# ilovin/lstm_ctc_ocr

Hardware: AMD Instinct MI355X
Metric: captcha images/sec training (32x256, bs=64/GPU) (higher is better)
Workload: dtype bf16; 1 GPU; VGG-7 + BiLSTM(256) + CTC train step, H=32 W=256, 10-char labels, C=64, bs=64/GPU (BASELINE.json configs[1]), Adam lr 1e-4 wd 1e-5 clip 10; global_batch=64, parallelism=dp1, hipgraph=True

## Files before the change

include/ocr_hip.h:

```cpp
#ifndef OCR_HIP_H
#define OCR_HIP_H
#include <stddef.h>
#ifdef __cplusplus
extern "C" {
#endif

enum { OCR_STATUS_OK = 0, OCR_STATUS_MEMOPS = 1, OCR_STATUS_INVALID = 2, OCR_STATUS_EXEC = 3 };

enum {
    OCR_EPI_BIAS = 1, OCR_EPI_RELU = 2, OCR_EPI_OUT_F32 = 4,
    OCR_EPI_MASK = 16, OCR_EPI_ROWSWAP = 32, OCR_EPI_ACCUM = 64
};

const char* ocr_status_string(int status);
int ocr_abi_version(void);
const char* ocr_build_id(void);

int ocr_ctc_workspace_size(int max_label_len, int max_time, int minibatch, size_t* bytes);
int ocr_ctc_loss(const float* activations, float* gradients, const int* flat_labels, const int* label_lengths,
                 const int* input_lengths, int alphabet_size, int minibatch, int max_time, int max_label_len,
                 int blank_label, float* costs, void* workspace, void* stream);
int ocr_ctc_debug(void* dbg);
int ocr_ctc_train_supported(int alphabet_size, int max_time, int max_label_len);
int ocr_ctc_loss_train(const float* activations, void* grad_ntc_bf16, float scale, const int* flat_labels,
                       const int* label_lengths, const int* input_lengths, int alphabet_size, int minibatch, int max_time,
                       int max_label_len, int blank_label, float* costs, void* stream);
int ocr_set_ctc_engine(int fast);
int ocr_ctc_long_placement(int alphabet_size, int max_time, int max_label_len);
int ocr_ctc_long_supported(int alphabet_size, int max_time, int max_label_len);
int ocr_ctc_long_workspace_size(int alphabet_size, int max_label_len, int max_time, int minibatch, size_t* bytes);
int ocr_ctc_loss_long(const float* activations, float* gradients ,
                      void* grad_ntc_bf16 , float scale,
                      const int* flat_labels, const int* label_lengths, const int* input_lengths,
                      int alphabet_size, int minibatch, int max_time, int max_label_len, int blank_label,
                      float* costs, void* workspace, size_t workspace_bytes, void* stream);
int ocr_ctc_wide_supported(int alphabet_size, int max_time, int max_label_len);
int ocr_ctc_wide_workspace_size(int alphabet_size, int max_label_len, int max_time, int minibatch, size_t* bytes);
int ocr_ctc_loss_wide(const float* activations, float* gradients ,
                      void* grad_ntc_bf16 , float scale,
                      const int* flat_labels, const int* label_lengths, const int* input_lengths,
                      int alphabet_size, int minibatch, int max_time, int max_label_len, int blank_label,
                      float* costs, void* workspace, size_t workspace_bytes, void* stream);
int ocr_ctc_score_supported(int alphabet_size, int max_time, int max_label_len, int num_candidates);
int ocr_ctc_score_workspace_size(int alphabet_size, int max_time, int minibatch, size_t* bytes);
int ocr_ctc_score(const float* activations, const int* input_lengths, const int* cand_labels, const int* cand_lengths, int sample_stride,
                  int alphabet_size, int minibatch, int max_time, int num_candidates, int max_label_len, int blank_label,
                  float* costs, int* best, float* best_cost, float* log_norm, void* workspace, size_t workspace_bytes, void* stream);
int ocr_ctc_trie_chunk_capacity(void);
int ocr_ctc_trie_supported(int alphabet_size, int max_time, int num_words);
int ocr_ctc_trie_build(const int* words, const int* lengths, int num_words, int max_label_len, int alphabet_size, int blank_label,
                       int chunk_nodes, int* num_chunks, int* num_nodes, int* nodes, int* chunk_node_start, int* chunk_word_start,
                       int* word_node, int* word_index);
int ocr_ctc_trie_workspace_size(int alphabet_size, int max_time, int minibatch, size_t* bytes);
int ocr_ctc_score_trie(const float* activations, const int* input_lengths, const int* nodes, const int* chunk_node_start,
                       const int* chunk_word_start, const int* word_node, const int* word_index, int num_chunks, int chunk_nodes,
                       int alphabet_size, int minibatch, int max_time, int num_words, int blank_label, float* costs, int* best,
                       float* best_cost, float* log_norm, void* workspace, size_t workspace_bytes, void* stream);
int ocr_ctc_topk_supported(int K, int k);
int ocr_ctc_topk_plan(int N, int K, int k, int* segments, int* segment_len);
int ocr_ctc_topk_workspace_size(int N, int K, int k, size_t* bytes);
int ocr_ctc_topk(const float* costs, long ld, int N, int K, int k, const float* log_norm, int* index, float* cost, float* log_post,
                 int* count, void* workspace, size_t workspace_bytes, void* stream);
int ocr_ctc_align_supported(int alphabet_size, int max_time, int max_label_len, int num_candidates);
int ocr_ctc_align_workspace_size(int alphabet_size, int max_time, int minibatch, int num_candidates, int max_label_len, size_t* bytes);
int ocr_ctc_align(const float* activations, const int* input_lengths, const int* cand_labels, const int* cand_lengths, int sample_stride,
                  int alphabet_size, int minibatch, int max_time, int num_candidates, int max_label_len, int blank_label,
                  int* start, int* end, float* score, float* path_cost, void* workspace, size_t workspace_bytes, void* stream);
int ocr_ctc_greedy_decode(const float* activations, const int* input_lengths, int alphabet_size, int minibatch,
                          int max_time, int blank_label, int pad_value, int* decoded, int* decoded_lengths,
                          void* stream);

int ocr_ctc_beam_workspace_size(int alphabet_size, int minibatch, int max_time, int beam_width, size_t* bytes);
int ocr_ctc_beam_decode(const float* activations, const int* input_lengths, int alphabet_size, int minibatch,
                        int max_time, int beam_width, int merge_repeated, int pad_value, int* decoded,
                        int* decoded_lengths, float* neg_log_prob, void* workspace, size_t workspace_bytes, void* stream);
int ocr_ctc_beam_kernel_choice(int alphabet_size, int beam_width);
int ocr_set_beam_engine(int engine);

int ocr_gemm_nt_bf16(const void* P, long ldp, const void* Q, long ldq, void* out, long ldo, int M, int N, int K,
                     const float* bias, const void* mask, long ldmask, int flags, int splits, int row_group,
                     int row_skip, int swap_inner, int swap_outer, void* stream);
int ocr_set_gemm_engine(int use_large_tile);
int ocr_conv3x3_bf16(const void* x, const void* wpack, void* y, int Nb, int W, int H, int Cin, int Cout,
                     const float* bias, const void* mask, int flags, void* stream);
int ocr_conv3x3_stats_rows(int Nb, int W, int H, int Cin, int Cout, int flags);
int ocr_conv3x3_bf16_stats(const void* x, const void* wpack, void* y, int Nb, int W, int H, int Cin, int Cout, const float* bias, int flags,
                           float* partials, void* stream);
int ocr_conv3x3_kernel_choice(int Nb, int W, int H, int Cin, int Cout, int flags, int kw, int kh);
int ocr_conv3x3_accum_supported(int Nb, int W, int H, int Cin, int Cout);
int ocr_conv_halo_clock_debug(void* dbg);
int ocr_conv_ws_debug(void* dbg);
int ocr_conv3x3_pool_supported(int Nb, int W, int H, int Cin, int Cout, int kw, int kh);
int ocr_conv3x3_pool_codes_supported(int Nb, int W, int H, int Cin, int Cout, int kw, int kh);
int ocr_conv3x3_relu_pool_codes_bf16(const void* x, const void* wpack, void* y, void* pooled, void* codes, int Nb, int W, int H, int Cin,
                                     int Cout, const float* bias, int kw, int kh, void* stream);
int ocr_conv3x3_relu_pool_bf16(const void* x, const void* wpack, void* y, void* pooled, int Nb, int W, int H, int Cin, int Cout,
                               const float* bias, int kw, int kh, void* stream);
int ocr_conv3x3_unpool_supported(int Nb, int W, int H, int Cin, int Cout, int kw, int kh);
int ocr_conv3x3_dgrad_unpool_bf16(const void* dy, const void* wdgrad, void* out_full, const void* codes, int Nb, int W, int H, int Cin,
                                  int Cout, int kw, int kh, int relu_mask, void* stream);
int ocr_gemm_tn_bf16(const void* A, long lda, const void* B, long ldb, float* out, long ldo, int Mk, int I, int J,
                     int row_group, int row_skip, long a_row_off, float scale, int splits, float* colsum, void* stream);
long ocr_gemm_tn_split_workspace_floats(int Mk, int I, int J);
int ocr_gemm_tn_split_bf16(const void* A, long lda, const void* B, long ldb, float* out, long ldo, int Mk, int I, int J, float scale,
                           float* colsum, float* part, long part_floats, void* stream);
int ocr_gemm_tn_batched_bf16(const void* A, long lda, long strideA, const void* B, long ldb, long strideB, float* out, long ldo,
                             long strideOut, int Mk, int I, int J, int nbatch, float scale, int splits, float* colsum,
                             long strideColsum, void* stream);
typedef struct ocr_tn_job {
    const void* A; long lda; long strideA;
    const void* B; long ldb; long strideB;
    float* out; long ldo; long strideOut;
    float* colsum; long strideColsum;
    int Mk, I, J, nbatch;
    int row_group, row_skip;
    float scale; int reserved;
} ocr_tn_job;
int ocr_gemm_tn_jobs_supported(const ocr_tn_job* jobs, int njobs);
int ocr_gemm_tn_jobs_bf16(const ocr_tn_job* jobs, int njobs, void* stream);
int ocr_set_wgrad_engine(int engine);
int ocr_conv3x3_wgrad_bf16(const void* x, const void* dy, float* dw, float* dbias, int Nb, int W, int H, int Cin,
                           int Cout, int splits, void* stream);
int ocr_conv3x3_wgrad_kernel_choice(int Nb, int W, int H, int Cin, int Cout, int has_workspace, int splits);

int ocr_conv3x3_wgrad_workspace_size(int Nb, int W, int H, int Cin, int Cout, size_t* bytes);
int ocr_conv3x3_wgrad_ws_bf16(const void* x, const void* dy, float* dw, float* dbias, int Nb, int W, int H, int Cin,
                              int Cout, int splits, void* workspace, size_t workspace_bytes, void* stream);
int ocr_conv3x3_wgrad_defer_bf16(const void* x, const void* dy, float* dw, float* dbias, int Nb, int W, int H, int Cin, int Cout,
                                 void* workspace, size_t workspace_bytes, void* job, int* job_blocks, int* deferred, void* stream);
int ocr_wgrad9_reduce_jobs(const void* jobs, int njobs, int total_blocks, void* stream);
int ocr_conv3x3_wgrad_pair_supported(const int* shape_first, const int* shape_second);
int ocr_conv3x3_wgrad_pair_defer_bf16(const void* x0, const void* dy0, float* dw0, float* dbias0, const int* shape0, void* workspace0,
                                      size_t workspace_bytes0, const void* x1, const void* dy1, float* dw1, float* dbias1, const int* shape1,
                                      void* workspace1, size_t workspace_bytes1, void* job0, void* job1, int* job_blocks0, int* job_blocks1,
                                      void* stream);

int ocr_conv1_fwd(const float* x, const float* w, const float* bias, void* y, int Nb, int W, int H, int Cout,
                  int relu, void* stream);
int ocr_conv1_wgrad(const float* x, const void* dz, float* dw, float* db, int Nb, int W, int H, int Cout,
                    void* stream);
int ocr_eltwise_bf16(int op, const void* a, const void* b, void* out, long n, void* stream);
int ocr_conv1_pool_fwd(const float* x, const float* w, const float* bias, void* p, int Nb, int W, int H, int Cout, void* stream);
int ocr_conv1_pool_fwd_train(const float* x, const float* w, const float* bias, void* p, int Nb, int W, int H, int Cout,
                             void* codes, float* zero, long zero_n, void* ones, long ones_n, void* stream);
int ocr_conv1_pool_bwd_codes(const float* x, const float* w, const float* bias, const void* dp, float* dw, float* db,
                             int Nb, int W, int H, int Cout, const void* codes, void* stream);
int ocr_conv1_pool_bwd_slab_rows(int Nb, int W, int H);
int ocr_conv1_pool_bwd_slab(const float* x, const float* w, const float* bias, const void* dp, int Nb, int W, int H, int Cout,
                            const void* codes, float* slab, void* stream);
int ocr_conv1_pool_bwd(const float* x, const float* w, const float* bias, const void* dp, float* dw, float* db, int Nb,
                       int W, int H, int Cout, void* stream);
int ocr_maxpool_fwd(const void* x, void* y, int Nb, int W, int H, int C, int kw, int kh, void* stream);
int ocr_maxpool_bwd(const void* x, const void* dy, void* dx, int Nb, int W, int H, int C, int kw, int kh,
                    int relu_mask, void* stream);
int ocr_maxpool_bwd_codes(const void* codes, const void* dy, void* dx, int Nb, int W, int H, int C, int kw, int kh,
                          int relu_mask, void* stream);
size_t ocr_bn_workspace_bytes(long M, int C);
int ocr_bn_train_fwd(const void* x, void* y, const float* gamma, const float* beta, float* save_mean,
                     float* save_rstd, long M, int C, float eps, int relu, void* workspace, const void* residual, void* stream);
int ocr_bn_train_bwd(const void* x, const void* y, const void* dy, void* dx, const float* gamma,
                     const float* save_mean, const float* save_rstd, float* dgamma, float* dbeta, long M, int C,
                     int relu, void* workspace, void* stream);
int ocr_bn_train_fwd2(const void* x, void* y, const float* gamma, const float* beta, float* save_mean, float* save_rstd, long M, int C,
                      float eps, int relu, void* workspace, const void* residual, int partial_rows, void* pooled, void* stream);
int ocr_bn_train_bwd2(const void* x, const void* y, const void* dy, void* dx, const float* gamma, const float* save_mean,
                      const float* save_rstd, float* dgamma, float* dbeta, long M, int C, int relu, void* workspace, int pooled_dy,
                      int partial_rows, void* stream);
int ocr_bn_train_fwd_codes(const void* x, const float* gamma, const float* beta, float* save_mean, float* save_rstd, long M, int C,
                           float eps, int relu, void* workspace, int partial_rows, void* pooled, void* codes, void* stream);
int ocr_bn_train_bwd_codes(const void* x, const void* codes, const void* dy, void* dx, const float* gamma, const float* save_mean,
                           const float* save_rstd, float* dgamma, float* dbeta, long M, int C, int relu, void* workspace, void* stream);
int ocr_bn_train_bwd_codes_col(const void* x, const void* codes, const void* col, int Nb, int W, int HC, void* dy_pooled_out, void* dx,
                               const float* gamma, const float* save_mean, const float* save_rstd, float* dgamma, float* dbeta, long M,
                               int C, int relu, void* workspace, void* stream);
int ocr_conv3x3_bnbwd_rows(int Nb, int W, int H, int Cin, int Cout);
int ocr_conv3x3_dgrad_bnbwd_bf16(const void* dy, const void* wdgrad, void* dx, int Nb, int W, int H, int Cin, int Cout, const void* mask_y,
                                 const void* z, const float* mean, const float* rstd, float* partials, void* stream);
int ocr_colsum_bf16(const void* a, float* out, long M, int C, long lda, void* stream);
int ocr_pack_transpose(const float* in, void* out, int R, int Cc, long ldin, int lstm_units, void* stream);
int ocr_pack_conv_dgrad(const float* w, void* out, int Cin, int Cout, void* stream);
int ocr_pack_jobs(const void* jobs, int njobs, int total_blocks, void* stream);
int ocr_cast_f32_bf16(const float* in, void* out, long n, void* stream);
int ocr_u8_to_unit_f32(const void* in, float* out, long n, void* stream);
int ocr_step_report(const float* costs, int n, const double* scalars, const void* word_addrs, int nwords, double* out, void* stream);
int ocr_bind_batch(const void* pixels, int pixels_are_u8, float* x, long n_pixels, const int* seq_len, int* seq_len_dst, int n_seq,
                   const int* labels, int* labels_dst, int n_labels, const int* labels_len, int* labels_len_dst, int n_labels_len,
                   void* stream);
int ocr_cast2d_f32_bf16(const float* in, long ldin, void* out, long ldout, int rows, int cols, void* stream);
int ocr_tnc_to_ntc_bf16(const float* in, void* out, int T, int N, int C, float scale, void* stream);
int ocr_conv5_col2im(const void* col, void* dx, int Nb, int W, int HC, void* stream);

int ocr_bn_infer_fwd(const void* x, void* y, const float* gamma, const float* beta, const float* mean, const float* var,
                     long M, int C, float eps, int relu, void* stream);
int ocr_bn_infer_bwd(const void* x, const void* y, const void* dy, void* dx, const float* gamma, const float* mean,
                     const float* var, float* dgamma, float* dbeta, long M, int C, float eps, int relu, void* stream);
int ocr_dropout_bf16(const void* in, void* out, long n, unsigned seed, const void* step_counter, float keep_prob, void* stream);
int ocr_avgpool_bf16(const void* src, void* dst, int Nb, int W, int H, int C, int kw, int kh, int backward, void* stream);
int ocr_subsample_bf16(const void* src, void* dst, int Nb, int W, int H, int C, int Wo, int Ho, int sw, int sh, int ow, int oh,
                       int backward, void* stream);
int ocr_softmax_f32(const float* in, float* out, long rows, int C, void* stream);

int ocr_lstm_fwd_step(const float* xproj, const void* whT_packed, const int* seq_len, void* hout, float* gates,
                      float* cell, int Nb, int T, int U, int step, float forget_bias, int ndir, void* stream);
int ocr_lstm_bwd_step(const void* wh, long ldw, long w_dir_stride, const int* seq_len, const void* dhout,
                      const float* gates, const float* cell, void* dz, float* dc_state, int Nb, int T, int U,
                      int step, int ndir, void* stream);
int ocr_lstm_seq_supported(int Nb, int U);
long ocr_lstm_seq_sync_words(int Nb, int U);
int ocr_lstm_seq_debug(void* dbg );
int ocr_lstm_seq_test_skew(int units, int at);
int ocr_lstm_fwd_seq(const float* xproj, const void* whT_packed, const int* seq_len, void* hout, float* gates,
                     float* cell, int Nb, int T, int U, float forget_bias, void* sync, void* stream);
int ocr_lstm_bwd_seq(const void* wh, long ldw, long w_dir_stride, const int* seq_len, const void* dhout,
                     const float* gates, const float* cell, void* dz, int Nb, int T, int U, void* sync, void* stream);
#define OCR_LSTM_PREPARED 1
int ocr_lstm_fwd_seq2(const float* xproj, const void* whT_packed, const int* seq_len, void* hout, float* gates,
                      float* cell, int Nb, int T, int U, float forget_bias, void* sync, int flags, void* stream);
int ocr_lstm_bwd_seq2(const void* wh, long ldw, long w_dir_stride, const int* seq_len, const void* dhout,
                      const float* gates, const float* cell, void* dz, int Nb, int T, int U, void* sync, int flags, void* stream);
int ocr_lstm_fwd_seq_x_supported(int Nb, int U, int D);
int ocr_lstm_fwd_seq_x(const void* x, const void* wxT_packed, const float* bias_packed, int D, const void* whT_packed,
                       const int* seq_len, void* hout, float* gates, float* cell, int Nb, int T, int U, float forget_bias,
                       void* sync, int flags, void* stream);
int ocr_set_lstm_proto(int proto);
int ocr_set_lstm_ksplit(int waves);
int ocr_lstm_hprev(const void* hout, const int* seq_len, void* hprev, int Nb, int T, int U, int ndir, void* stream);
int ocr_lstm_xh(const void* x, const void* hout, const int* seq_len, void* xh, int Nb, int T, int D, int U, int ndir, void* stream);
int ocr_lstm_pack_bias(const float* b_fw, const float* b_bw , float* out, int U, int ndir, void* stream);

int ocr_optim_scalar_count(void);
int ocr_optim_init(void* scalars , double lr, void* stream);
int ocr_optim_set_lr(void* scalars, double lr, int multiply, void* stream);
int ocr_optim_step(float* params, float* grads, float* state1, float* state2, long n, long reg_begin, long reg_end,
                   float weight_decay, float clip_norm, int solver, float beta1, float beta2, float eps,
                   void* scalars, void* stream);
int ocr_optim_step_guarded(float* params, float* grads, float* state1, float* state2, long n, long reg_begin, long reg_end,
                           float weight_decay, float clip_norm, int solver, float beta1, float beta2, float eps,
                           void* scalars, const void* guard_addrs, int nguard, void* stream);
int ocr_optim_step_guarded2(float* params, float* grads, float* state1, float* state2, long n, long reg_begin, long reg_end,
                            float weight_decay, float clip_norm, int solver, float beta1, float beta2, float eps,
                            void* scalars, const void* guard_addrs, int nguard, const float* drop_flag, void* stream);
int ocr_guard_flag(const void* guard_addrs, int nguard, float* flag_out, void* stream);

int ocr_captcha_synth(const int* params, int n_images, int words_per_image, int max_glyphs, const void* atlas, const int* stamp, int n_stamp,
                      void* out, int W, int out_h, int canvas_cap, int width_cap, void* stream);

int ocr_wgrad9_debug(void* dbg);

int ocr_probe_tr16(const int* addr , int* out , void* stream);
int ocr_probe_xcc(int* out , int nblocks, int threads, void* stream);
int ocr_occupy_cus(int nblocks, int threads, int lds_bytes, float us, void* stream);
int ocr_mfma_busy_probe(float* out, int nblocks, int threads , int iters, long long* clk, void* stream);

#ifdef __cplusplus
}
#endif
#endif
```

lstm_ctc_ocr_amd/_native.py:

```python
import ctypes
import os
import re

_HERE = os.path.dirname(os.path.abspath(__file__))
LIB_PATH = os.environ.get("OCR_NATIVE_LIB") or os.path.join(_HERE, "libocrhip.so")
HEADER_PATH = os.path.join(os.path.dirname(_HERE), "include", "ocr_hip.h")

EPI_BIAS, EPI_RELU, EPI_OUT_F32, EPI_MASK, EPI_ROWSWAP, EPI_ACCUM = 1, 2, 4, 16, 32, 64

_P, _I, _L, _F, _D = ctypes.c_void_p, ctypes.c_int, ctypes.c_long, ctypes.c_float, ctypes.c_double

_SIGS = {
    "ocr_abi_version": ([], _I),
    "ocr_build_id": ([], ctypes.c_char_p),
    "ocr_status_string": ([_I], ctypes.c_char_p),
    "ocr_ctc_workspace_size": ([_I, _I, _I, ctypes.POINTER(ctypes.c_size_t)], _I),
    "ocr_ctc_loss": ([_P, _P, _P, _P, _P, _I, _I, _I, _I, _I, _P, _P, _P], _I),
    "ocr_set_ctc_engine": ([_I], _I),
    "ocr_ctc_debug": ([_P], _I),
    "ocr_ctc_train_supported": ([_I, _I, _I], _I),
    "ocr_ctc_loss_train": ([_P, _P, _F, _P, _P, _P, _I, _I, _I, _I, _I, _P, _P], _I),
    "ocr_ctc_long_placement": ([_I, _I, _I], _I),
    "ocr_ctc_long_supported": ([_I, _I, _I], _I),
    "ocr_ctc_long_workspace_size": ([_I, _I, _I, _I, ctypes.POINTER(ctypes.c_size_t)], _I),
    "ocr_ctc_loss_long": ([_P, _P, _P, _F, _P, _P, _P, _I, _I, _I, _I, _I, _P, _P, ctypes.c_size_t, _P], _I),
    "ocr_ctc_wide_supported": ([_I, _I, _I], _I),
    "ocr_ctc_wide_workspace_size": ([_I, _I, _I, _I, ctypes.POINTER(ctypes.c_size_t)], _I),
    "ocr_ctc_loss_wide": ([_P, _P, _P, _F, _P, _P, _P, _I, _I, _I, _I, _I, _P, _P, ctypes.c_size_t, _P], _I),
    "ocr_ctc_score_supported": ([_I, _I, _I, _I], _I),
    "ocr_ctc_score_workspace_size": ([_I, _I, _I, ctypes.POINTER(ctypes.c_size_t)], _I),
    "ocr_ctc_score": ([_P, _P, _P, _P, _I, _I, _I, _I, _I, _I, _I, _P, _P, _P, _P, _P, ctypes.c_size_t, _P], _I),
    "ocr_ctc_trie_chunk_capacity": ([], _I),
    "ocr_ctc_trie_supported": ([_I, _I, _I], _I),
    "ocr_ctc_trie_build": ([_P, _P, _I, _I, _I, _I, _I, ctypes.POINTER(_I), ctypes.POINTER(_I), _P, _P, _P, _P, _P], _I),
    "ocr_ctc_trie_workspace_size": ([_I, _I, _I, ctypes.POINTER(ctypes.c_size_t)], _I),
    "ocr_ctc_score_trie": ([_P, _P, _P, _P, _P, _P, _P, _I, _I, _I, _I, _I, _I, _I, _P, _P, _P, _P, _P, ctypes.c_size_t, _P], _I),
    "ocr_ctc_topk_supported": ([_I, _I], _I),
    "ocr_ctc_topk_plan": ([_I, _I, _I, ctypes.POINTER(_I), ctypes.POINTER(_I)], _I),
    "ocr_ctc_topk_workspace_size": ([_I, _I, _I, ctypes.POINTER(ctypes.c_size_t)], _I),
    "ocr_ctc_topk": ([_P, _L, _I, _I, _I, _P, _P, _P, _P, _P, _P, ctypes.c_size_t, _P], _I),
    "ocr_ctc_align_supported": ([_I, _I, _I, _I], _I),
    "ocr_ctc_align_workspace_size": ([_I, _I, _I, _I, _I, ctypes.POINTER(ctypes.c_size_t)], _I),
    "ocr_ctc_align": ([_P, _P, _P, _P, _I, _I, _I, _I, _I, _I, _I, _P, _P, _P, _P, _P, ctypes.c_size_t, _P], _I),
    "ocr_ctc_greedy_decode":([_P, _P, _I, _I, _I, _I, _I, _P, _P, _P], _I),
    "ocr_ctc_beam_workspace_size": ([_I, _I, _I, _I, ctypes.POINTER(ctypes.c_size_t)], _I),
    "ocr_ctc_beam_decode": ([_P, _P, _I, _I, _I, _I, _I, _I, _P, _P, _P, _P, ctypes.c_size_t, _P], _I),
    "ocr_ctc_beam_kernel_choice": ([_I, _I], _I),
    "ocr_set_beam_engine": ([_I], _I),
    "ocr_gemm_nt_bf16": ([_P, _L, _P, _L, _P, _L, _I, _I, _I, _P, _P, _L, _I, _I, _I, _I, _I, _I, _P], _I),
    "ocr_set_gemm_engine": ([_I], _I),
    "ocr_gemm_tn_batched_bf16": ([_P, _L, _L, _P, _L, _L, _P, _L, _L, _I, _I, _I, _I, _F, _I, _P, _L, _P], _I),
    "ocr_gemm_tn_jobs_supported": ([_P, _I], _I),
    "ocr_gemm_tn_jobs_bf16": ([_P, _I, _P], _I),
    "ocr_lstm_xh": ([_P, _P, _P, _P, _I, _I, _I, _I, _I, _P], _I),
    "ocr_set_wgrad_engine": ([_I], _I),
    "ocr_conv3x3_bf16": ([_P, _P, _P, _I, _I, _I, _I, _I, _P, _P, _I, _P], _I),
    "ocr_conv_halo_clock_debug": ([_P], _I),
    "ocr_occupy_cus": ([_I, _I, _I, _F, _P], _I),
    "ocr_conv_ws_debug": ([_P], _I),
    "ocr_conv3x3_accum_supported": ([_I, _I, _I, _I, _I], _I),
    "ocr_conv3x3_kernel_choice": ([_I, _I, _I, _I, _I, _I, _I, _I], _I),
    "ocr_conv3x3_pool_supported": ([_I, _I, _I, _I, _I, _I, _I], _I),
    "ocr_conv3x3_relu_pool_bf16": ([_P, _P, _P, _P, _I, _I, _I, _I, _I, _P, _I, _I, _P], _I),
    "ocr_conv3x3_pool_codes_supported": ([_I, _I, _I, _I, _I, _I, _I], _I),
    "ocr_conv3x3_relu_pool_codes_bf16": ([_P, _P, _P, _P, _P, _I, _I, _I, _I, _I, _P, _I, _I, _P], _I),
    "ocr_gemm_tn_bf16": ([_P, _L, _P, _L, _P, _L, _I, _I, _I, _I, _I, _L, _F, _I, _P, _P], _I),
    "ocr_gemm_tn_split_workspace_floats": ([_I, _I, _I], _L),
    "ocr_gemm_tn_split_bf16": ([_P, _L, _P, _L, _P, _L, _I, _I, _I, _F, _P, _P, _L, _P], _I),
    "ocr_conv3x3_wgrad_bf16": ([_P, _P, _P, _P, _I, _I, _I, _I, _I, _I, _P], _I),
    "ocr_conv3x3_wgrad_kernel_choice": ([_I, _I, _I, _I, _I, _I, _I], _I),
    "ocr_conv3x3_wgrad_workspace_size": ([_I, _I, _I, _I, _I, ctypes.POINTER(ctypes.c_size_t)], _I),
    "ocr_conv3x3_wgrad_ws_bf16": ([_P, _P, _P, _P, _I, _I, _I, _I, _I, _I, _P, ctypes.c_size_t, _P], _I),
    "ocr_conv3x3_wgrad_defer_bf16": ([_P, _P, _P, _P, _I, _I, _I, _I, _I, _P, ctypes.c_size_t, _P, ctypes.POINTER(_I),
                                      ctypes.POINTER(_I), _P], _I),
    "ocr_conv3x3_wgrad_pair_supported": ([ctypes.POINTER(_I), ctypes.POINTER(_I)], _I),
    "ocr_conv3x3_wgrad_pair_defer_bf16": ([_P, _P, _P, _P, ctypes.POINTER(_I), _P, ctypes.c_size_t, _P, _P, _P, _P, ctypes.POINTER(_I), _P,
                                           ctypes.c_size_t, _P, _P, ctypes.POINTER(_I), ctypes.POINTER(_I), _P], _I),
    "ocr_wgrad9_reduce_jobs": ([_P, _I, _I, _P], _I),
    "ocr_conv1_fwd": ([_P, _P, _P, _P, _I, _I, _I, _I, _I, _P], _I),
    "ocr_conv1_wgrad": ([_P, _P, _P, _P, _I, _I, _I, _I, _P], _I),
    "ocr_eltwise_bf16": ([_I, _P, _P, _P, _L, _P], _I),
    "ocr_conv1_pool_fwd": ([_P, _P, _P, _P, _I, _I, _I, _I, _P], _I),
    "ocr_conv1_pool_fwd_train": ([_P, _P, _P, _P, _I, _I, _I, _I, _P, _P, _L, _P, _L, _P], _I),
    "ocr_conv1_pool_bwd_codes": ([_P, _P, _P, _P, _P, _P, _I, _I, _I, _I, _P, _P], _I),
    "ocr_conv1_pool_bwd_slab_rows": ([_I, _I, _I], _I),
    "ocr_conv1_pool_bwd_slab": ([_P, _P, _P, _P, _I, _I, _I, _I, _P, _P, _P], _I),
    "ocr_conv1_pool_bwd": ([_P, _P, _P, _P, _P, _P, _I, _I, _I, _I, _P], _I),
    "ocr_maxpool_fwd": ([_P, _P, _I, _I, _I, _I, _I, _I, _P], _I),
    "ocr_maxpool_bwd": ([_P, _P, _P, _I, _I, _I, _I, _I, _I, _I, _P], _I),
    "ocr_bn_workspace_bytes": ([_L, _I], ctypes.c_size_t),
    "ocr_bn_train_fwd": ([_P, _P, _P, _P, _P, _P, _L, _I, _F, _I, _P, _P, _P], _I),
    "ocr_bn_train_bwd": ([_P, _P, _P, _P, _P, _P, _P, _P, _P, _L, _I, _I, _P, _P], _I),
    "ocr_bn_train_fwd2": ([_P, _P, _P, _P, _P, _P, _L, _I, _F, _I, _P, _P, _I, _P, _P], _I),
    "ocr_bn_train_bwd2": ([_P, _P, _P, _P, _P, _P, _P, _P, _P, _L, _I, _I, _P, _I, _I, _P], _I),
    "ocr_maxpool_bwd_codes": ([_P, _P, _P, _I, _I, _I, _I, _I, _I, _I, _P], _I),
    "ocr_bn_train_fwd_codes": ([_P, _P, _P, _P, _P, _L, _I, _F, _I, _P, _I, _P, _P, _P], _I),
    "ocr_bn_train_bwd_codes": ([_P, _P, _P, _P, _P, _P, _P, _P, _P, _L, _I, _I, _P, _P], _I),
    "ocr_bn_train_bwd_codes_col": ([_P, _P, _P, _I, _I, _I, _P, _P, _P, _P, _P, _P, _P, _L, _I, _I, _P, _P], _I),
    "ocr_conv3x3_unpool_supported": ([_I, _I, _I, _I, _I, _I, _I], _I),
    "ocr_conv3x3_dgrad_unpool_bf16": ([_P, _P, _P, _P, _I, _I, _I, _I, _I, _I, _I, _I, _P], _I),
    "ocr_conv3x3_bnbwd_rows": ([_I, _I, _I, _I, _I], _I),
    "ocr_conv3x3_dgrad_bnbwd_bf16": ([_P, _P, _P, _I, _I, _I, _I, _I, _P, _P, _P, _P, _P, _P], _I),
    "ocr_conv3x3_stats_rows": ([_I, _I, _I, _I, _I, _I], _I),
    "ocr_conv3x3_bf16_stats": ([_P, _P, _P, _I, _I, _I, _I, _I, _P, _I, _P, _P], _I),
    "ocr_bn_infer_fwd": ([_P, _P, _P, _P, _P, _P, _L, _I, _F, _I, _P], _I),
    "ocr_bn_infer_bwd": ([_P, _P, _P, _P, _P, _P, _P, _P, _P, _L, _I, _F, _I, _P], _I),
    "ocr_dropout_bf16": ([_P, _P, _L, ctypes.c_uint, _P, _F, _P], _I),
    "ocr_avgpool_bf16": ([_P, _P, _I, _I, _I, _I, _I, _I, _I, _P], _I),
    "ocr_subsample_bf16": ([_P, _P, _I, _I, _I, _I, _I, _I, _I, _I, _I, _I, _I, _P], _I),
    "ocr_softmax_f32": ([_P, _P, _L, _I, _P], _I),
    "ocr_colsum_bf16": ([_P, _P, _L, _I, _L, _P], _I),
    "ocr_pack_transpose": ([_P, _P, _I, _I, _L, _I, _P], _I),
    "ocr_pack_conv_dgrad": ([_P, _P, _I, _I, _P], _I),
    "ocr_pack_jobs": ([_P, _I, _I, _P], _I),
    "ocr_cast_f32_bf16": ([_P, _P, _L, _P], _I),
    "ocr_u8_to_unit_f32": ([_P, _P, _L, _P], _I),
    "ocr_step_report": ([_P, _I, _P, _P, _I, _P, _P], _I),
    "ocr_bind_batch": ([_P, _I, _P, _L, _P, _P, _I, _P, _P, _I, _P, _P, _I, _P], _I),
    "ocr_captcha_synth": ([_P, _I, _I, _I, _P, _P, _I, _P, _I, _I, _I, _I, _P], _I),
    "ocr_cast2d_f32_bf16": ([_P, _L, _P, _L, _I, _I, _P], _I),
    "ocr_tnc_to_ntc_bf16": ([_P, _P, _I, _I, _I, _F, _P], _I),
    "ocr_conv5_col2im": ([_P, _P, _I, _I, _I, _P], _I),
    "ocr_lstm_fwd_step": ([_P, _P, _P, _P, _P, _P, _I, _I, _I, _I, _F, _I, _P], _I),
    "ocr_lstm_bwd_step": ([_P, _L, _L, _P, _P, _P, _P, _P, _P, _I, _I, _I, _I, _I, _P], _I),
    "ocr_lstm_seq_supported": ([_I, _I], _I),
    "ocr_lstm_seq_debug": ([_P], _I),
    "ocr_lstm_seq_test_skew": ([_I, _I], _I),
    "ocr_lstm_seq_sync_words": ([_I, _I], _L),
    "ocr_lstm_fwd_seq": ([_P, _P, _P, _P, _P, _P, _I, _I, _I, _F, _P, _P], _I),
    "ocr_lstm_bwd_seq": ([_P, _L, _L, _P, _P, _P, _P, _P, _I, _I, _I, _P, _P], _I),
    "ocr_lstm_fwd_seq2": ([_P, _P, _P, _P, _P, _P, _I, _I, _I, _F, _P, _I, _P], _I),
    "ocr_lstm_fwd_seq_x_supported": ([_I, _I, _I], _I),
    "ocr_lstm_fwd_seq_x": ([_P, _P, _P, _I, _P, _P, _P, _P, _P, _I, _I, _I, _F, _P, _I, _P], _I),
    "ocr_lstm_bwd_seq2": ([_P, _L, _L, _P, _P, _P, _P, _P, _I, _I, _I, _P, _I, _P], _I),
    "ocr_lstm_hprev": ([_P, _P, _P, _I, _I, _I, _I, _P], _I),
    "ocr_lstm_pack_bias": ([_P, _P, _P, _I, _I, _P], _I),
    "ocr_optim_scalar_count": ([], _I),
    "ocr_optim_init": ([_P, _D, _P], _I),
    "ocr_optim_set_lr": ([_P, _D, _I, _P], _I),
    "ocr_optim_step": ([_P, _P, _P, _P, _L, _L, _L, _F, _F, _I, _F, _F, _F, _P, _P], _I),
    "ocr_optim_step_guarded": ([_P, _P, _P, _P, _L, _L, _L, _F, _F, _I, _F, _F, _F, _P, _P, _I, _P], _I),
    "ocr_optim_step_guarded2": ([_P, _P, _P, _P, _L, _L, _L, _F, _F, _I, _F, _F, _F, _P, _P, _I, _P, _P], _I),
    "ocr_guard_flag": ([_P, _I, _P, _P], _I),
    "ocr_wgrad9_debug": ([_P], _I),
    "ocr_probe_tr16": ([_P, _P, _P], _I),
    "ocr_set_lstm_proto": ([_I], _I),
    "ocr_set_lstm_ksplit": ([_I], _I),
    "ocr_probe_xcc": ([_P, _I, _I, _P], _I),
    "ocr_mfma_busy_probe": ([_P, _I, _I, _I, _P, _P], _I),
}


class NativeError(RuntimeError):
    pass


def declared_symbols(header=HEADER_PATH):
    text = open(header).read()
    text = re.sub(r"/\*.*?\*/", "", text, flags=re.S)
    return sorted(set(re.findall(r"\b(ocr_[a-z0-9_]+)\s*\(", text)))


def source_build_id(csrc=os.path.join(_HERE, "csrc"), experiments=False):
    import glob
    import hashlib
    rel = [os.path.basename(f) for f in glob.glob(os.path.join(csrc, "*.hip"))]
    h = hashlib.sha256()
    for f in sorted(rel) + ["common.h", "conv_plan.h", "ctc_common.h", "Makefile"]:
        h.update(open(os.path.join(csrc, f), "rb").read())
    return h.hexdigest()[:16] + ("-exp" if experiments else "")


def build_id():
    return lib().ocr_build_id().decode()


_lib = None


def lib():
    global _lib
    if _lib is None:
        if not os.path.exists(LIB_PATH):
            raise NativeError(
                "libocrhip.so not found at %s — build it with `python -c 'import __graft_entry__ as g; g.build()'` "
                "(there is no CPU/eager fallback for the hot path)" % LIB_PATH)
        _lib = ctypes.CDLL(LIB_PATH)
        for name, (argtypes, restype) in _SIGS.items():
            fn = getattr(_lib, name)
            fn.argtypes = argtypes
            fn.restype = restype
        for env, setter in (("OCR_GEMM_ENGINE", "ocr_set_gemm_engine"), ("OCR_WGRAD_ENGINE", "ocr_set_wgrad_engine")):
            if os.environ.get(env):
                getattr(_lib, setter)(int(os.environ[env]))
    return _lib


def status_string(code):
    return lib().ocr_status_string(code).decode()


def call(name, *args):
    rc = getattr(lib(), name)(*args)
    if rc != 0:
        raise NativeError("%s failed: status %d (%s)" % (name, rc, status_string(rc)))


def ptr(t):
    return None if t is None else t.data_ptr()


def stream():
    import torch
    return torch.cuda.current_stream().cuda_stream
```

lstm_ctc_ocr_amd/csrc/gemm.hip:

```cpp
#include "conv_plan.h"
#include <string.h>

enum {
    EPI_BIAS = 1,
    EPI_RELU = 2,
    EPI_OUT_F32 = 4,
    EPI_ATOMIC = 8,
    EPI_MASK = 16,
    EPI_ROWSWAP = 32,
    EPI_ACCUM = 64,
};

struct GemmArgs {
    const bf16_t* P;
    const bf16_t* Q;
    long ldp, ldq;
    int M, N, K;
    int k_per_split;
    int grp, skip;
    int cW, cH, cC;
    void* out;
    long ldo;
    const float* bias;
    const bf16_t* mask;
// ... 60 lines not shown
                int kc = k0 + ((tid + i * 256) & 3) * 8;
                u32x4 v = {0, 0, 0, 0};
                if (pvalid[i] && kc < kend) v = *(const u32x4*)(prow[i] + k0);
                pst[i] = v;
            }
        } else {
            int tap = k0 / g.cC;
            int ci0 = k0 - tap * g.cC;
            int dw = tap / 3 - 1, dh = tap % 3 - 1;
            long shift = ((long)dw * g.cH + dh) * g.cC + ci0;
#pragma unroll
            for (int i = 0; i < NCP; ++i) {
                int ww = pw[i] + dw, hh = ph[i] + dh;
                bool ok = pvalid[i] && (unsigned)ww < (unsigned)g.cW && (unsigned)hh < (unsigned)g.cH;
                u32x4 v = {0, 0, 0, 0};
                if (ok) v = *(const u32x4*)(prow[i] + shift);
                pst[i] = v;
            }
        }
#pragma unroll
        for (int i = 0; i < NCQ; ++i) {
            int kc = k0 + ((tid + i * 256) & 3) * 8;
            u32x4 v = {0, 0, 0, 0};
            if (qvalid[i] && kc < kend) v = *(const u32x4*)(qrow[i] + k0);
            qst[i] = v;
        }
    };
    auto store_tiles = [&]() {
#pragma unroll
        for (int i = 0; i < NCP; ++i) {
            int c = tid + i * 256;
            *(u32x4*)(&Ps[(c >> 2) * LDS_ROW + (c & 3) * 8]) = pst[i];
        }
#pragma unroll
        for (int i = 0; i < NCQ; ++i) {
            int c = tid + i * 256;
            *(u32x4*)(&Qs[(c >> 2) * LDS_ROW + (c & 3) * 8]) = qst[i];
        }
    };

    f32x4 acc[FN][FM];
#pragma unroll
    for (int a = 0; a < FN; ++a)
#pragma unroll
        for (int b = 0; b < FM; ++b) acc[a][b] = (f32x4){0.f, 0.f, 0.f, 0.f};

    const int frow = lane & 15, fk = (lane >> 4) * 8;
    if (kbeg < kend) {
        load_tiles(kbeg);
        for (int k0 = kbeg; k0 < kend; k0 += 32) {
            __syncthreads();
            store_tiles();
            __syncthreads();
            if (k0 + 32 < kend) load_tiles(k0 + 32);
            bf16x8 af[FN], bfr[FM];
#pragma unroll
            for (int a = 0; a < FN; ++a)
                af[a] = *(const bf16x8*)(&Qs[(wn * 16 * FN + a * 16 + frow) * LDS_ROW + fk]);
#pragma unroll
            for (int b = 0; b < FM; ++b)
                bfr[b] = *(const bf16x8*)(&Ps[(wm * 16 * FM + b * 16 + frow) * LDS_ROW + fk]);
#pragma unroll
            for (int a = 0; a < FN; ++a)
#pragma unroll
                for (int b = 0; b < FM; ++b)
                    acc[a][b] = __builtin_amdgcn_mfma_f32_16x16x32_bf16(af[a], bfr[b], acc[a][b], 0, 0, 0);
        }
    }

    const int flags = g.flags;
    const bool add_bias = (flags & EPI_BIAS) && (!(flags & EPI_ATOMIC) || blockIdx.z == 0);
#pragma unroll
    for (int a = 0; a < FN; ++a) {
        int n = n0 + wn * 16 * FN + a * 16 + (lane >> 4) * 4;
        if (n >= g.N) continue;
        f32x4 bv = {0.f, 0.f, 0.f, 0.f};
        if (add_bias) bv = *(const f32x4*)(g.bias + n);
#pragma unroll
        for (int b = 0; b < FM; ++b) {
            int m = m0 + wm * 16 * FM + b * 16 + (lane & 15);
            if (m >= g.M) continue;
            f32x4 v = acc[a][b] + bv;
            if (flags & EPI_RELU) {
                v.x = fmaxf(v.x, 0.f); v.y = fmaxf(v.y, 0.f); v.z = fmaxf(v.z, 0.f); v.w = fmaxf(v.w, 0.f);
            }
            if (flags & EPI_MASK) {
                u32x2 mk = *(const u32x2*)(g.mask + (long)m * g.ldmask + n);
                if (!(bf_lo(mk.x) > 0.f)) v.x = 0.f;
                if (!(bf_hi(mk.x) > 0.f)) v.y = 0.f;
                if (!(bf_lo(mk.y) > 0.f)) v.z = 0.f;
                if (!(bf_hi(mk.y) > 0.f)) v.w = 0.f;
            }
            long orow = m;
            if (flags & EPI_ROWSWAP) orow = (long)(m % g.swap_inner) * g.swap_outer + m / g.swap_inner;
            if (flags & EPI_OUT_F32) {
                float* o = (float*)g.out + orow * g.ldo + n;
                if (flags & EPI_ATOMIC) {
                    atomicAdd(o + 0, v.x); atomicAdd(o + 1, v.y); atomicAdd(o + 2, v.z); atomicAdd(o + 3, v.w);
                } else if (flags & EPI_ACCUM) {
                    f32x4 old = *(f32x4*)o;
                    *(f32x4*)o = old + v;
                } else {
                    *(f32x4*)o = v;
                }
            } else {
                u32x2 pk;
                pk.x = pack_bf2(v.x, v.y);
                pk.y = pack_bf2(v.z, v.w);
                *(u32x2*)((bf16_t*)g.out + orow * g.ldo + n) = pk;
            }
        }
    }
}

template <int MODE, int FM, int FN>
static int launch_gemm(const GemmArgs& g, hipStream_t stream) {
    constexpr int BM = 32 * FM, BN = 32 * FN;
    int splits = ceil_div(g.K, g.k_per_split);
    dim3 grid(ceil_div(g.M, BM), ceil_div(g.N, BN), splits);
    gemm_nt_kernel<MODE, FM, FN><<<grid, 256, 0, stream>>>(g);
    OCR_CHECK_LAUNCH();
    return OCR_OK;
}

static int dispatch_gemm(GemmArgs& g, int mode, int splits, hipStream_t stream) {
    if (g.M <= 0 || g.N <= 0 || g.K <= 0 || (g.K & 7) || (g.N & 3)) return OCR_ERR_INVALID;
    if (!g.P || !g.Q || !g.out) return OCR_ERR_INVALID;
    if (splits < 1) splits = 1;
    int kps = ceil_div(ceil_div(g.K, splits), 32) * 32;
    g.k_per_split = kps;
    if (splits > 1) {
        if (!(g.flags & EPI_OUT_F32) || (g.flags & (EPI_RELU | EPI_MASK | EPI_ACCUM))) return OCR_ERR_INVALID;
        g.flags |= EPI_ATOMIC;
    }
    long big_blocks = (long)ceil_div(g.M, 128) * ceil_div(g.N, 128) * ceil_div(g.K, kps);
    bool big = big_blocks >= 192 && g.N >= 128;
    if (mode == 1) {
        if (g.cC % 32 || g.K != 9 * g.cC) return OCR_ERR_INVALID;
        return big ? launch_gemm<1, 4, 4>(g, stream) : launch_gemm<1, 2, 2>(g, stream);
    }
    return big ? launch_gemm<0, 4, 4>(g, stream) : launch_gemm<0, 2, 2>(g, stream);
}

int ig_try_dispatch(const void* P, long ldp, const void* Q, long ldq, void* out, long ldo, int M, int N, int K,
                    const float* bias, const void* mask, long ldmask, int flags, int mode, int grp, int skip, int cW,
                    int cH, int cC, int swap_inner, int swap_outer, hipStream_t stream);
static int g_use_igemm = 1, g_use_halo = 1;
extern int g_ig_stages;
extern "C" int ocr_set_gemm_engine(int mode) {
    if (mode < 0 || mode > 3) return OCR_ERR_INVALID;
    g_use_igemm = mode != 0; g_use_halo = mode == 1; g_ig_stages = (mode == 2) ? 2 : 3;
    return OCR_OK;
}

extern "C" int ocr_gemm_nt_bf16(const void* P, long ldp, const void* Q, long ldq, void* out, long ldo,
                                int M, int N, int K, const float* bias, const void* mask, long ldmask,
                                int flags, int splits, int row_group, int row_skip, int swap_inner,
                                int swap_outer, void* stream) {
    GemmArgs g = {};
    g.P = (const bf16_t*)P; g.Q = (const bf16_t*)Q; g.ldp = ldp; g.ldq = ldq;
    g.M = M; g.N = N; g.K = K; g.grp = row_group; g.skip = row_skip;
    g.out = out; g.ldo = ldo; g.bias = bias; g.mask = (const bf16_t*)mask; g.ldmask = ldmask;
    g.flags = flags & ~EPI_ATOMIC; g.swap_inner = swap_inner; g.swap_outer = swap_outer;
    if ((flags & EPI_BIAS) && !bias) return OCR_ERR_INVALID;
    if ((flags & EPI_MASK) && !mask) return OCR_ERR_INVALID;
    if ((flags & EPI_ROWSWAP) && (swap_inner <= 0 || swap_outer <= 0)) return OCR_ERR_INVALID;
    if (g_use_igemm && splits <= 1 && P && Q && out && M > 0 && N > 0 && K > 0) {
        int rc = ig_try_dispatch(P, ldp, Q, ldq, out, ldo, M, N, K, bias, mask, ldmask, g.flags, 0, row_group, row_skip, 0, 0, 0,
                                 swap_inner, swap_outer, (hipStream_t)stream);
        if (rc >= 0) return rc;
    }
    return dispatch_gemm(g, 0, splits, (hipStream_t)stream);
}


struct ConvKnobs {
    int ws, k2, k3, k2_cfg;
    int k2_minsteps, k2_mintiles, k2_allow_a, k2_abl, k2_nst;
    int k3_minsteps, k3_genw, k3_prio;
    int halo_nw, halo_stagger, halo_stagger_bit, halo_prio;
};
static int env_int(const char* e, int dflt) { return e ? atoi(e) : dflt; }
static ConvKnobs read_conv_knobs() {
    ConvKnobs k;
    k.ws = env_int(getenv("OCR_CONV_WS"), 1);
    k.k2 = env_int(getenv("OCR_CONV_K2"), 1);
    k.k3 = env_int(getenv("OCR_CONV_K3"), 1);
    const char* cfg = getenv("OCR_K2_CFG");
    k.k2_cfg = (cfg && (cfg[0] == 'A' || cfg[0] == 'D')) ? cfg[0] : 0;
    k.k2_minsteps = env_int(ocr_tune_env("OCR_K2_MINSTEPS"), 18);
    k.k2_mintiles = env_int(ocr_tune_env("OCR_K2_MINTILES"), 128);
    const char* tiles = ocr_tune_env("OCR_K2_TILES");
    k.k2_allow_a = !(tiles && tiles[0] == 'D');
    k.k2_abl = env_int(ocr_tune_env("OCR_K2_ABL"), 0);
    k.k2_nst = env_int(ocr_tune_env("OCR_K2_NST"), 0);
    k.k3_minsteps = env_int(ocr_tune_env("OCR_K3_MINSTEPS"), 18);
    k.k3_genw = env_int(ocr_tune_env("OCR_K3_GENW"), 1);
    k.k3_prio = env_int(ocr_tune_env("OCR_K3_PRIO"), 2);
    k.halo_nw = env_int(ocr_tune_env("OCR_HALO_NW"), 0);
    const char* st = ocr_tune_env("OCR_HALO_STAGGER");
    const char* comma = st ? strchr(st, ',') : nullptr;
    k.halo_stagger = st && atoi(st) > 0 ? atoi(st) : 0;
    k.halo_stagger_bit = comma ? atoi(comma + 1) : 32;
    k.halo_prio = env_int(ocr_tune_env("OCR_HALO_PRIO"), 1);
    return k;
}
static const ConvKnobs& conv_knobs() {
    static const ConvKnobs k = read_conv_knobs();
    return k;
}

int ocr_cu_count() {
    static int cus = 0;
    if (!cus) {
        int dev = 0; hipDeviceProp_t prop;
        if (hipGetDevice(&dev) == hipSuccess && hipGetDeviceProperties(&prop, dev) == hipSuccess && prop.multiProcessorCount > 0) cus = prop.multiProcessorCount;
    }
    return cus > 0 ? cus : 256;
}

static bool plan_ws(ConvPlan& p, const ConvKnobs& k) {
    if (!k.ws || (p.flags & ~(EPI_BIAS | EPI_RELU | EPI_MASK))) return false;
    if (p.epi_kind && (!(p.flags & EPI_RELU) || (p.flags & EPI_MASK))) return false;
    if ((p.Cout & 63) || (long)p.M * p.Cin * 2 > 0x7fffffffL || (long)p.M * p.Cout * 2 > 0x7fffffffL) return false;
    int nc, bm;
    if (p.H == 16 && p.Cin == 64) { nc = 16; bm = 256; }
    else if (p.H == 16 && p.Cin == 128) { nc = 8; bm = 128; }
    else if (p.H == 8 && p.Cin == 128) { nc = 16; bm = 128; }
    else return false;
    if (p.W % nc || p.M % bm || (p.epi_kind == CONV_EPI_POOL22 && (p.W & 1))) return false;
    const int ncu = ocr_cu_count();
    const int mtiles = p.M / bm, ntiles = p.Cout / 64;
    if (k.ws == 1 && (p.Cin != 64 || (long)mtiles * ntiles < 2L * ncu)) return false;
    int slots = ncu / ntiles;
    if (slots < 1) slots = 1;
    if (slots > mtiles) slots = mtiles;
    p.per_slot = (mtiles + slots - 1) / slots;
    p.slots = (mtiles + p.per_slot - 1) / p.per_slot;
    p.grid = p.slots * ntiles;
    p.xcd_map = (p.grid % 8 == 0 && (p.grid / 8) % ntiles == 0) ? 1 : 0;
    p.family = CONV_WS; p.ws_nc = nc; p.ws_ksplit = p.Cin == 64 ? 1 : 2;
    return true;
}

static char k2_tile(const ConvPlan& p, const ConvKnobs& k, int minsteps) {
    const long M = p.M;
    if ((p.Cin & 63) || (p.Cout & 63) || M < 4096 || p.H > 16 || p.H < 1) return 0;
    if (M * p.Cin * 2 >= 0x7fffffffL || (long)p.Cout * 9 * p.Cin * 2 >= 0x7fffffffL) return 0;
    for (int pass = 0; pass < 2; ++pass)
        for (const char c : {'A', 'D'}) {
            if (k.k2_cfg && c != k.k2_cfg) continue;
            if (!k.k2_cfg && c == 'A' && !k.k2_allow_a) continue;
            const int bn = c == 'A' ? 128 : 64;
            if (p.Cout % bn) continue;
            if (k.k2_cfg) return c;
            if (9 * (p.Cin / 64) < minsteps) return 0;
            if ((M + 255) / 256 * (p.Cout / bn) >= (pass == 0 ? 224 : k.k2_mintiles)) return c;
        }
    return 0;
}

static bool plan_k3(ConvPlan& p, const ConvKnobs& k, char tile) {
    const int H = p.H, epi = p.epi_kind;
    if (H != 2 && H != 4 && H != 8 && H != 16) return false;
    if (p.M % 256 || (p.Cin & 63) || (p.Cout & 63) || (tile == 'A' && p.Cout % 128)) return false;
    const int NC = 256 / H, PS = (NC + 2 + 7) / 8 * 8;
    const bool genw = p.W % NC != 0;
    if (genw && (H == 16 || NC + 2 + (NC + p.W - 1) / p.W > PS)) return false;
    if (genw && !k.k3_genw) return false;
    if (H == 2 && (!genw || epi == CONV_EPI_POOL12 || epi == CONV_EPI_POOL22)) return false;
    if (epi >= CONV_EPI_STATS && (p.flags & EPI_ACCUM)) return false;
    if (epi == CONV_EPI_BNBWD && (!(p.flags & EPI_MASK) || p.Cin == 64 || (H != 4 && H != 8))) return false;
    p.family = CONV_K3; p.tile = tile; p.genw = genw; p.single = H == 16 && p.Cin == 64; p.prio = k.k3_prio;
    return true;
}

static bool plan_k3_k2(ConvPlan& p, const ConvKnobs& k) {
    if (k.k3) {
        const char t = k2_tile(p, k, k.k3_minsteps >= 0 ? k.k3_minsteps : k.k2_minsteps);
        if (t && plan_k3(p, k, t)) return true;
    }
    if (p.epi_kind >= CONV_EPI_STATS) return false;
    const char t = k2_tile(p, k, k.k2_minsteps);
    if (!t) return false;
    int nst = t == 'A' ? 5 : 4;
    if ((t == 'A' && k.k2_nst == 4) || (t == 'D' && (k.k2_nst == 5 || k.k2_nst == 6))) nst = k.k2_nst;
    const int FM = t == 'A' ? 8 : 4, BN = t == 'A' ? 128 : 64;
    const int NRpad = (256 + 2 * p.H + 4 + 7) / 8 * 8;
    const int lds = 2 * NRpad * 128 + nst * BN * 128;
    if (lds > 163840 || lds < 8 * FM * 2048) return false;
#ifdef OCR_EXPERIMENTS
    if (lds + 10240 > 163840 && (k.k2_abl & 8)) return false;
#endif
    p.family = CONV_K2; p.tile = t; p.nst = nst; p.abl = k.k2_abl;
    return true;
}

static bool plan_halo(ConvPlan& p, const ConvKnobs& k) {
    const int H = p.H, Cout = p.Cout, nw = k.halo_nw;
    p.prio = k.halo_prio; p.stagger = k.halo_stagger; p.stagger_bit = k.halo_stagger_bit;
    if (nw != 8) {
        const int NR = 128 + 2 * H + 2, NRp = (NR + 32) / 32 * 32;
        const long mt4 = (p.M + 127) / 128;
        if (NRp / 32 == 5 || NRp / 32 == 6) {
            p.family = CONV_HALO; p.nw = 4; p.bn = (Cout >= 128 && mt4 * ((Cout + 127) / 128) >= 448) ? 128 : 64;
            return true;
// ... 149 lines not shown
```

lstm_ctc_ocr_amd/csrc/gemm_tn3.hip:

```cpp
#include "common.h"
#include <stdlib.h>
#include <type_traits>

struct Tn3Job {
    const bf16_t* A; long lda; long sA;
    const bf16_t* B; long ldb; long sB;
    float* out; long ldo; long sO;
    float* colsum; long sC;
    int Mk, I, J, nbatch;
    int grp, skip;
    float scale; int reserved;
};
static_assert(sizeof(Tn3Job) == 120, "mirrored by lstm_ctc_ocr_amd/ops.py (ctypes.Structure)");

__device__ u32x4 tn3_zero_page[4];

typedef const __attribute__((address_space(1))) void* gptr_t;
typedef __attribute__((address_space(3))) void* lptr_t;
typedef __attribute__((ext_vector_type(4))) short s16x4;
typedef __attribute__((ext_vector_type(8))) short s16x8;

__device__ __forceinline__ int tn3_frag_off(int cb, int lane) {
    const int g = lane >> 4, L = lane & 15;
    const int r0 = 4 * g + (L >> 2);
    const int q = cb * 2 + ((L & 3) >> 1);
    const int p = q ^ ((r0 & 7) << 1);
    return r0 * 256 + p * 16 + (L & 1) * 8;
}

template <int KH, int NST >
__device__ __forceinline__ void tn3_body(const Tn3Job& g, const int bid, unsigned char* smem) {
    constexpr int TILE = 64 * 256, STAGE = 2 * TILE, DEPTH = NST - 2;
    const int tid = threadIdx.x, lane = tid & 63;
    const int wave = __builtin_amdgcn_readfirstlane(tid >> 6);
    const int wi = (wave & 3) >> 1, wj = wave & 1;

    const int IT = g.I >> 7, JT = g.J >> 7, T = IT * JT * g.nbatch;
    int L = bid;
    if ((T & 7) == 0) L = (bid & 7) * (T >> 3) + (bid >> 3);
    int jt, it;
    if ((long)g.I >= (long)g.J) { jt = L % JT; it = (L / JT) % IT; }
    else { it = L % IT; jt = (L / IT) % JT; }
    const int bi = L / (JT * IT);
    const bf16_t* A = g.A + (long)bi * g.sA;
    const bf16_t* B = g.B + (long)bi * g.sB;
    float* out = g.out + (long)bi * g.sO;
    const int i0 = it * 128, j0 = jt * 128, Mk = g.Mk;
    const bool do_cs = g.colsum != nullptr && it == 0;
    const bf16_t* zero = (const bf16_t*)tn3_zero_page;

    const int rsub = lane >> 4, pos = lane & 15;
    const bf16_t* pa[2]; const bf16_t* pb[2];
    int mrow[2], mq[2], mr[2];
    const int grp = g.grp, dq = grp > 0 ? 64 / grp : 0, dr = grp > 0 ? 64 % grp : 0;
#pragma unroll
    for (int j = 0; j < 2; ++j) {
        const int r = (wave * 2 + j) * 4 + rsub;
        const int q = pos ^ ((r & 7) << 1);
        mrow[j] = r;
        mq[j] = grp > 0 ? r / grp : 0; mr[j] = grp > 0 ? r % grp : 0;
        pa[j] = A + i0 + q * 8;
        pb[j] = B + j0 + q * 8;
    }
    auto stage_load = [&](int buf) {
        unsigned char* sa = smem + buf * STAGE;
        unsigned char* sb = sa + TILE;
#pragma unroll
        for (int j = 0; j < 2; ++j) {
            const int m = mrow[j];
            const bf16_t* srca = zero;
            const bf16_t* srcb = zero;
            if (m < Mk) {
                srca = pa[j] + ((long)m + (long)mq[j] * g.skip) * g.lda;
                srcb = pb[j] + (long)m * g.ldb;
            }
            __builtin_amdgcn_global_load_lds((gptr_t)srca, (lptr_t)(sa + (wave * 2 + j) * 1024), 16, 0, 0);
            __builtin_amdgcn_global_load_lds((gptr_t)srcb, (lptr_t)(sb + (wave * 2 + j) * 1024), 16, 0, 0);
            mrow[j] = m + 64;
            if (grp > 0) {
                int r2 = mr[j] + dr, q2 = mq[j] + dq;
                if (r2 >= grp) { r2 -= grp; ++q2; }
                mr[j] = r2; mq[j] = q2;
            }
        }
    };

    f32x4 acc[4][4];
#pragma unroll
    for (int a = 0; a < 4; ++a)
#pragma unroll
        for (int b = 0; b < 4; ++b) acc[a][b] = (f32x4){0.f, 0.f, 0.f, 0.f};
    float cs[8] = {0.f, 0.f, 0.f, 0.f, 0.f, 0.f, 0.f, 0.f};

    const unsigned lds0 = (unsigned)(size_t)(lptr_t)smem;
    unsigned offf[8];
#pragma unroll
    for (int a = 0; a < 4; ++a) {
        offf[a] = lds0 + tn3_frag_off(wi * 4 + a, lane) + KH * 32 * 256;
        offf[4 + a] = lds0 + TILE + tn3_frag_off(wj * 4 + a, lane) + KH * 32 * 256;
    }

    const int nst = (Mk + 63) >> 6;
#pragma unroll
    for (int d = 0; d < DEPTH; ++d) stage_load(d);
    asm volatile("s_waitcnt vmcnt(0)" ::: "memory");
    __builtin_amdgcn_s_barrier();
    asm volatile("" ::: "memory");

    s16x4 flo[8], fhi[8];
    auto load = [&](int buf) {
#pragma unroll
        for (int f = 0; f < 8; ++f) {
            const unsigned ad = offf[f] + buf * STAGE;
            asm volatile("ds_read_b64_tr_b16 %0, %1" : "=v"(flo[f]) : "v"(ad));
            asm volatile("ds_read_b64_tr_b16 %0, %1 offset:4096" : "=v"(fhi[f]) : "v"(ad));
        }
    };
    auto comp = [&]() {
        asm volatile("s_waitcnt lgkmcnt(0)" ::: "memory");
        __builtin_amdgcn_sched_barrier(0);
        __builtin_amdgcn_s_setprio(KH == 1 ? 2 : 1);
        bf16x8 fr[8];
#pragma unroll
        for (int f = 0; f < 8; ++f) {
            s16x8 v = {flo[f][0], flo[f][1], flo[f][2], flo[f][3], fhi[f][0], fhi[f][1], fhi[f][2], fhi[f][3]};
            fr[f] = __builtin_bit_cast(bf16x8, v);
        }
#pragma unroll
        for (int a = 0; a < 4; ++a)
#pragma unroll
            for (int b = 0; b < 4; ++b)
                acc[a][b] = __builtin_amdgcn_mfma_f32_16x16x32_bf16(fr[a], fr[4 + b], acc[a][b], 0, 0, 0);
        __builtin_amdgcn_s_setprio(0);
        __builtin_amdgcn_sched_barrier(0);
    };
    int buf = 0;
    for (int s = 0; s < nst; ++s) {
        int nb = buf + DEPTH; if (nb >= NST) nb -= NST;
        if (KH == 0) {
            load(buf);
            stage_load(nb);
            comp();
            if (do_cs) {
                const unsigned tb = lds0 + buf * STAGE + TILE;
                const int q = tid & 15;
                u32x4 v[4];
#pragma unroll
                for (int i = 0; i < 4; ++i) {
                    const int r = (tid >> 4) + 16 * i;
                    asm volatile("ds_read_b128 %0, %1" : "=v"(v[i]) : "v"(tb + r * 256 + ((q ^ ((r & 7) << 1)) << 4)));
                }
                asm volatile("s_waitcnt lgkmcnt(0)" ::: "memory");
                __builtin_amdgcn_sched_barrier(0);
#pragma unroll
                for (int i = 0; i < 4; ++i) {
                    cs[0] += bf_lo(v[i].x); cs[1] += bf_hi(v[i].x); cs[2] += bf_lo(v[i].y); cs[3] += bf_hi(v[i].y);
                    cs[4] += bf_lo(v[i].z); cs[5] += bf_hi(v[i].z); cs[6] += bf_lo(v[i].w); cs[7] += bf_hi(v[i].w);
                }
            }
        } else {
            if (s > 0) comp();
            load(buf);
            stage_load(nb);
        }
        asm volatile("s_waitcnt vmcnt(%0)" ::"n"(4 * (DEPTH - 1)) : "memory");
        __builtin_amdgcn_sched_barrier(0);
        __builtin_amdgcn_s_barrier();
        asm volatile("" ::: "memory");
        __builtin_amdgcn_sched_barrier(0);
        buf = (buf + 1 == NST) ? 0 : buf + 1;
    }
    if (KH == 1) comp();
    asm volatile("s_waitcnt vmcnt(0)" ::: "memory");
    __syncthreads();

    {
        f32x4* mine = (f32x4*)smem + (size_t)wave * (8 * 64);
        const f32x4* theirs = (const f32x4*)smem + (size_t)(wave ^ 4) * (8 * 64);
#pragma unroll
        for (int a2 = 0; a2 < 2; ++a2)
#pragma unroll
            for (int b = 0; b < 4; ++b) mine[(a2 * 4 + b) * 64 + lane] = acc[(1 - KH) * 2 + a2][b];
        __syncthreads();
#pragma unroll
        for (int a2 = 0; a2 < 2; ++a2)
#pragma unroll
            for (int b = 0; b < 4; ++b) acc[KH * 2 + a2][b] += theirs[(a2 * 4 + b) * 64 + lane];
    }
    if (do_cs) {
        __syncthreads();
        float* red = (float*)smem;
        if (KH == 0) {
#pragma unroll
            for (int e = 0; e < 8; ++e) red[tid * 8 + e] = cs[e];
        }
        __syncthreads();
        if (tid < 128) {
            float t = 0.f;
            for (int u = tid >> 3; u < 256; u += 16) t += red[u * 8 + (tid & 7)];
            g.colsum[(long)bi * g.sC + j0 + tid] += t * g.scale;
        }
    }
    const float scale = g.scale;
    float old[2][4][4];
#pragma unroll
    for (int a2 = 0; a2 < 2; ++a2)
#pragma unroll
        for (int b = 0; b < 4; ++b)
#pragma unroll
            for (int r = 0; r < 4; ++r)
                old[a2][b][r] = __builtin_nontemporal_load(out + (long)(i0 + wi * 64 + (KH * 2 + a2) * 16 + (lane >> 4) * 4 + r) * g.ldo + j0 + wj * 64 + b * 16 + (lane & 15));
#pragma unroll
    for (int a2 = 0; a2 < 2; ++a2)
#pragma unroll
        for (int b = 0; b < 4; ++b)
#pragma unroll
            for (int r = 0; r < 4; ++r)
                out[(long)(i0 + wi * 64 + (KH * 2 + a2) * 16 + (lane >> 4) * 4 + r) * g.ldo + j0 + wj * 64 + b * 16 + (lane & 15)] =
                    old[a2][b][r] + acc[KH * 2 + a2][b][r] * scale;
}

template <int NST>
__global__ __launch_bounds__(512) __attribute__((amdgpu_waves_per_eu(2, 2))) void gemm_tn3_kernel(Tn3Job j0, Tn3Job j1, int nblk0) {
    extern __shared__ __attribute__((aligned(16))) unsigned char smem[];
    const int kh = __builtin_amdgcn_readfirstlane((int)(threadIdx.x >> 8));
    const int bid = (int)blockIdx.x;
    if (bid < nblk0) {
        if (kh == 0) tn3_body<0, NST>(j0, bid, smem); else tn3_body<1, NST>(j0, bid, smem);
    } else {
        if (kh == 0) tn3_body<0, NST>(j1, bid - nblk0, smem); else tn3_body<1, NST>(j1, bid - nblk0, smem);
    }
}

static bool tn3_covers(const Tn3Job& j) {
    if (!j.A || !j.B || !j.out || j.Mk < 256 || j.I <= 0 || j.J <= 0 || (j.I & 127) || (j.J & 127) || j.nbatch < 1) return false;
    if ((j.lda & 7) || (j.ldb & 7) || (j.sA & 7) || (j.sB & 7) || ((size_t)j.A & 15) || ((size_t)j.B & 15)) return false;
    if (j.grp < 0 || j.skip < 0 || (j.grp == 0 && j.skip != 0)) return false;
    return (long)(j.I >> 7) * (j.J >> 7) * j.nbatch <= 0x7fffffL;
}
extern "C" int ocr_gemm_tn_jobs_supported(const void* jobs, int njobs) {
    if (!jobs || njobs < 1 || njobs > 2) return 0;
    const Tn3Job* j = (const Tn3Job*)jobs;
    for (int k = 0; k < njobs; ++k) if (!tn3_covers(j[k])) return 0;
    return 1;
}
extern "C" int ocr_gemm_tn_jobs_bf16(const void* jobs, int njobs, void* stream) {
    if (!ocr_gemm_tn_jobs_supported(jobs, njobs)) return OCR_ERR_INVALID;
    const Tn3Job* j = (const Tn3Job*)jobs;
    const int t0 = (j[0].I >> 7) * (j[0].J >> 7) * j[0].nbatch;
    const int t1 = njobs > 1 ? (j[1].I >> 7) * (j[1].J >> 7) * j[1].nbatch : 0;
    static int nst = -1;
    if (nst < 0) { const char* e = getenv("OCR_TN3_NST"); nst = (e && atoi(e) == 5) ? 5 : 4; }
    const int lds = nst * 2 * 64 * 256;
    if (nst == 4) {
        if (ocr_allow_lds<gemm_tn3_kernel<4>>(lds) != hipSuccess) return OCR_ERR_EXEC;
        gemm_tn3_kernel<4><<<t0 + t1, 512, lds, (hipStream_t)stream>>>(j[0], njobs > 1 ? j[1] : j[0], t0);
    } else {
        if (ocr_allow_lds<gemm_tn3_kernel<5>>(lds) != hipSuccess) return OCR_ERR_EXEC;
        gemm_tn3_kernel<5><<<t0 + t1, 512, lds, (hipStream_t)stream>>>(j[0], njobs > 1 ? j[1] : j[0], t0);
    }
    OCR_CHECK_LAUNCH();
    return OCR_OK;
}
```

lstm_ctc_ocr_amd/csrc/igemm.hip:

```cpp
#include "common.h"
#include <stdlib.h>

enum { IG_BIAS = 1, IG_RELU = 2, IG_OUT_F32 = 4, IG_MASK = 16, IG_ROWSWAP = 32 };

struct IgArgs {
    const bf16_t* P; const bf16_t* Q;
    long ldp, ldq;
    int M, N, K;
    int grp, skip;
    int cW, cH, cC;
    void* out; long ldo;
    const float* bias; const bf16_t* mask; long ldmask;
    int flags, swap_inner, swap_outer;
};

__device__ u32x4 ig_zero_page[4];

typedef const __attribute__((address_space(1))) void* gptr_t;
typedef __attribute__((address_space(3))) void* lptr_t;

template <int BN, int MODE , int STAGES , int NW >
__global__ __launch_bounds__(64 * NW) __attribute__((amdgpu_waves_per_eu(2, 2))) void igemm_kernel(IgArgs g) {
    constexpr int BM = 32 * NW, BK = 64;
    constexpr int WAVES_N = BN / 64, WAVES_M = NW / WAVES_N;
    constexpr int WM = BM / WAVES_M;
    constexpr int FM = WM / 16, FN = 4;
    constexpr int PB = BM * BK * 2, QB = BN * BK * 2, STAGE = PB + QB;
    constexpr int QI = BN / (8 * NW);
    extern __shared__ __attribute__((aligned(16))) unsigned char smem[];

    const int tid = threadIdx.x, lane = tid & 63;
    const int wave = __builtin_amdgcn_readfirstlane(tid >> 6);
    const int wm = wave / WAVES_N, wn = wave % WAVES_N;

    const int mtiles = (g.M + BM - 1) / BM, ntiles = (g.N + BN - 1) / BN;
    const int nblk = mtiles * ntiles;
    int L = blockIdx.x;
    if ((nblk & 7) == 0) L = (L & 7) * (nblk >> 3) + (L >> 3);
    const int m0 = (L / ntiles) * BM, n0 = (L % ntiles) * BN;

    const int rsub = lane >> 3;
    const int csrc = ((lane & 7) ^ rsub) * 8;
    const bf16_t* zero = (const bf16_t*)ig_zero_page;
    const bf16_t* prow[4];
    int pw[4], ph[4];
    bool pok[4];
#pragma unroll
    for (int j = 0; j < 4; ++j) {
        int m = m0 + (wave * 4 + j) * 8 + rsub;
        pok[j] = m < g.M;
        int mm = pok[j] ? m : 0;
        if (MODE == 0) {
            long phys = (long)mm + (g.grp > 0 ? (long)(mm / g.grp) * g.skip : 0);
            prow[j] = g.P + phys * g.ldp + csrc;
            pw[j] = ph[j] = 0;
        } else {
            ph[j] = mm % g.cH;
            pw[j] = (mm / g.cH) % g.cW;
            prow[j] = g.P + (long)mm * g.cC + csrc;
        }
    }
    const bf16_t* qrow[QI];
#pragma unroll
    for (int j = 0; j < QI; ++j) {
        int n = n0 + (wave * QI + j) * 8 + rsub;
        qrow[j] = (n < g.N) ? g.Q + (long)n * g.ldq + csrc : nullptr;
    }

    auto stage_load = [&](int k0, int buf) {
        unsigned char* sp = smem + buf * STAGE;
        long shift = k0;
        int dw = 0, dh = 0;
        if (MODE == 1) {
            int tap = k0 / g.cC;
            dw = tap / 3 - 1; dh = tap % 3 - 1;
            shift = ((long)dw * g.cH + dh) * g.cC + (k0 - tap * g.cC);
        }
#pragma unroll
        for (int j = 0; j < 4; ++j) {
            bool ok = pok[j];
            if (MODE == 1) ok = ok && (unsigned)(pw[j] + dw) < (unsigned)g.cW && (unsigned)(ph[j] + dh) < (unsigned)g.cH;
            const bf16_t* src = ok ? prow[j] + shift : zero;
            __builtin_amdgcn_global_load_lds((gptr_t)src, (lptr_t)(sp + (wave * 4 + j) * 1024), 16, 0, 0);
        }
#pragma unroll
        for (int j = 0; j < QI; ++j) {
            const bf16_t* src = qrow[j] ? qrow[j] + k0 : zero;
            __builtin_amdgcn_global_load_lds((gptr_t)src, (lptr_t)(sp + PB + (wave * QI + j) * 1024), 16, 0, 0);
        }
    };

    f32x4 acc[FN][FM];
#pragma unroll
    for (int a = 0; a < FN; ++a)
#pragma unroll
        for (int b = 0; b < FM; ++b) acc[a][b] = (f32x4){0.f, 0.f, 0.f, 0.f};

    const int frow = lane & 15, fq = lane >> 4, fx = lane & 7;
    const int ntk = g.K / BK;
    constexpr int NI = 4 + QI;
    const unsigned lds0 = (unsigned)(size_t)(lptr_t)smem;
    const unsigned qoff = PB + (wn * 64 + frow) * 128 + ((fq ^ fx) << 4);
    const unsigned poff = (wm * WM + frow) * 128 + ((fq ^ fx) << 4);
    auto compute = [&](int buf) {
        const unsigned base = lds0 + buf * STAGE;
        u32x4 af[2][FN], bfr[2][FM];
#pragma unroll
        for (int kk = 0; kk < 2; ++kk) {
#pragma unroll
            for (int a = 0; a < FN; ++a)
                asm volatile("ds_read_b128 %0, %1 offset:%2" : "=v"(af[kk][a]) : "v"(base + (qoff ^ (kk * 64))), "n"(a * 2048));
#pragma unroll
            for (int b = 0; b < FM; ++b)
                asm volatile("ds_read_b128 %0, %1 offset:%2" : "=v"(bfr[kk][b]) : "v"(base + (poff ^ (kk * 64))), "n"(b * 2048));
        }
#pragma unroll
        for (int kk = 0; kk < 2; ++kk) {
            if (kk == 0) asm volatile("s_waitcnt lgkmcnt(%0)" ::"n"(FN + FM) : "memory");
            else asm volatile("s_waitcnt lgkmcnt(0)" ::: "memory");
            __builtin_amdgcn_sched_barrier(0);
#pragma unroll
            for (int a = 0; a < FN; ++a)
#pragma unroll
                for (int b = 0; b < FM; ++b)
                    acc[a][b] = __builtin_amdgcn_mfma_f32_16x16x32_bf16(__builtin_bit_cast(bf16x8, af[kk][a]),
                                                                        __builtin_bit_cast(bf16x8, bfr[kk][b]), acc[a][b], 0, 0, 0);
            __builtin_amdgcn_sched_barrier(0);
        }
    };
    if (STAGES == 2) {
        stage_load(0, 0);
        asm volatile("s_waitcnt vmcnt(0)" ::: "memory");
        __syncthreads();
        for (int t = 0; t < ntk; ++t) {
            const int cur = t & 1;
            if (t + 1 < ntk) stage_load((t + 1) * BK, cur ^ 1);
            compute(cur);
            asm volatile("s_waitcnt vmcnt(0)" ::: "memory");
            __syncthreads();
        }
    } else {
        stage_load(0, 0);
        if (ntk > 1) stage_load(BK, 1);
        int cur = 0;
        for (int t = 0; t < ntk; ++t) {
            if (t + 1 < ntk) asm volatile("s_waitcnt vmcnt(%0)" ::"n"(NI) : "memory");
            else asm volatile("s_waitcnt vmcnt(0)" ::: "memory");
            __builtin_amdgcn_s_barrier();
            asm volatile("" ::: "memory");
            if (t + 2 < ntk) { int nb = cur + 2; if (nb >= 3) nb -= 3; stage_load((t + 2) * BK, nb); }
            compute(cur);
            asm volatile("s_waitcnt lgkmcnt(0)" ::: "memory");
            cur = (cur == 2) ? 0 : cur + 1;
        }
    }

    const int flags = g.flags;
    f32x4 bv[FN];
#pragma unroll
    for (int a = 0; a < FN; ++a) {
        const int n = n0 + wn * 64 + a * 16 + (lane >> 4) * 4;
        bv[a] = (f32x4){0.f, 0.f, 0.f, 0.f};
        if ((flags & IG_BIAS) && n < g.N) bv[a] = *(const f32x4*)(g.bias + n);
    }
#pragma unroll
    for (int b = 0; b < FM; ++b) {
        const int m = m0 + wm * WM + b * 16 + (lane & 15);
        if (m >= g.M) continue;
        long orow = m;
        if (flags & IG_ROWSWAP) orow = (long)(m % g.swap_inner) * g.swap_outer + m / g.swap_inner;
#pragma unroll
        for (int a = 0; a < FN; ++a) {
            const int n = n0 + wn * 64 + a * 16 + (lane >> 4) * 4;
            if (n >= g.N) continue;
            f32x4 v = acc[a][b] + bv[a];
            if (flags & IG_RELU) {
                v.x = fmaxf(v.x, 0.f); v.y = fmaxf(v.y, 0.f); v.z = fmaxf(v.z, 0.f); v.w = fmaxf(v.w, 0.f);
            }
            if (flags & IG_MASK) {
                u32x2 mk = *(const u32x2*)(g.mask + (long)m * g.ldmask + n);
                if (!(bf_lo(mk.x) > 0.f)) v.x = 0.f;
                if (!(bf_hi(mk.x) > 0.f)) v.y = 0.f;
                if (!(bf_lo(mk.y) > 0.f)) v.z = 0.f;
                if (!(bf_hi(mk.y) > 0.f)) v.w = 0.f;
            }
            if (flags & IG_OUT_F32) {
                *(f32x4*)((float*)g.out + orow * g.ldo + n) = v;
            } else {
                u32x2 pk;
                pk.x = pack_bf2(v.x, v.y);
                pk.y = pack_bf2(v.z, v.w);
                *(u32x2*)((bf16_t*)g.out + orow * g.ldo + n) = pk;
            }
        }
    }
}

int g_ig_stages = 3;

template <int BN, int MODE, int STAGES, int NW>
static int launch_ig2(const IgArgs& g, hipStream_t stream) {
    constexpr int BM = 32 * NW;
    constexpr int LDS = STAGES * (BM * 128 + BN * 128);
    if (ocr_allow_lds<igemm_kernel<BN, MODE, STAGES, NW>>(LDS) != hipSuccess) return OCR_ERR_EXEC;
    int mt = (g.M + BM - 1) / BM, nt = (g.N + BN - 1) / BN;
    igemm_kernel<BN, MODE, STAGES, NW><<<mt * nt, 64 * NW, LDS, stream>>>(g);
    OCR_CHECK_LAUNCH();
    return OCR_OK;
}
template <int BN, int MODE>
static int launch_ig(const IgArgs& g, hipStream_t stream) {
    if (BN <= 128 && g_ig_stages == 3) return launch_ig2<(BN <= 128 ? BN : 128), MODE, 3, 8>(g, stream);
    return launch_ig2<BN, MODE, 2, 8>(g, stream);
}

int ig_try_dispatch(const void* P, long ldp, const void* Q, long ldq, void* out, long ldo, int M, int N, int K,
                    const float* bias, const void* mask, long ldmask, int flags, int mode, int grp, int skip, int cW,
                    int cH, int cC, int swap_inner, int swap_outer, hipStream_t stream) {
    if ((K & 63) || (N & 3) || M < 1024) return -1;
    if (mode == 1 && (cC & 63)) return -1;
    if (flags & ~(IG_BIAS | IG_RELU | IG_OUT_F32 | IG_MASK | IG_ROWSWAP)) return -1;
    IgArgs g = {};
    g.P = (const bf16_t*)P; g.Q = (const bf16_t*)Q; g.ldp = ldp; g.ldq = ldq; g.M = M; g.N = N; g.K = K;
    g.grp = grp; g.skip = skip; g.cW = cW; g.cH = cH; g.cC = cC; g.out = out; g.ldo = ldo; g.bias = bias;
    g.mask = (const bf16_t*)mask; g.ldmask = ldmask; g.flags = flags; g.swap_inner = swap_inner; g.swap_outer = swap_outer;
    static int ig_nw = -1;
    if (ig_nw < 0) { const char* e = ocr_tune_env("OCR_IG_NW"); ig_nw = e ? atoi(e) : 0; }
    if (mode == 0 && ig_nw != 8) {
        const long mt4 = (M + 127) / 128;
        const long wg8 = (long)((M + 255) / 256) * ((N + 127) / 128);
        if (ig_nw == 4 || wg8 < 400) {
            if (N >= 128 && mt4 * ((N + 127) / 128) >= 448) return launch_ig2<128, 0, 2, 4>(g, stream);
            return launch_ig2<64, 0, 3, 4>(g, stream);
        }
    }
    const int mt = (M + 255) / 256;
    int bn = 64;
    if (N >= 256 && (long)mt * ((N + 255) / 256) >= 256) bn = 256;
    else if (N >= 128 && (long)mt * ((N + 127) / 128) >= 256) bn = 128;
    else if (N >= 128 && (long)mt * ((N + 63) / 64) < 96) bn = 128;
#define IG_CASE(BNV)                                                                  \
    if (bn == BNV) return mode == 1 ? launch_ig<BNV, 1>(g, stream) : launch_ig<BNV, 0>(g, stream);
    IG_CASE(256) IG_CASE(128) IG_CASE(64)
#undef IG_CASE
    return -1;
}
```

lstm_ctc_ocr_amd/engine.py:

```python
import time

import numpy as np
import torch

from . import dist as ocr_dist
from . import ops
from ._native import NativeError, call as nat_call
from .engine_ops import (BF16, F32, I32, _env, _number, _switch, _AddOp, _AvgPoolOp, _BatchNormOp, _BiLstmOp, _ConcatOp, _ConvOp,
                         _Conv3x3Op, _DropoutOp, _FcOp, _InputOp, _PoolOp, _ReluOp, _SoftmaxOp, _SubsampleOp, _ViewOp, _conv_op)
from .lexicon import LexiconTrie
from .layout import FlatLayout, execution_order, init_host_parameters

ALIGN = 64





class ShapePlan(object):

    def _init_fields(self, N, W):
        self.N, self.W = N, W
        self.buf, self.shape = {}, {}
        self.scratch = {}
        self.dy_done = set()
        self.w9_pending, self.w9_tables = [], {}
        self.w9_pending_bytes = 0
        self.tn_pending = []
        self.w9_held = None
        self.tn_side_open = False
        self.fused_pools = set()
        self.bn_stat_rows = {}
        self.bn_bwd_rows = {}
        self.w9_hold_for = {}
        self.unpool_pools = set()
        self.col_bn = {}
        self.lstm_sync_keys = ()
        self.lstm_arena, self.lstm_sync = None, ()
        self.rings_ready, self.rings_armed = set(), False
        self.graph_fb = self.graph_fwd = self.graph_fb1 = self.graph_fb2 = self.graph_dp = self.graph_step = None
        self._guard_addrs = None
        self._report = None

    def __init__(self, eng, N, W):
        self._init_fields(N, W)
        dev = eng.device
        self.x = torch.zeros((N, W, eng.num_features), dtype=F32, device=dev)
        self.labels = torch.zeros(N * eng.max_label_len, dtype=I32, device=dev)
        self.labels_len = torch.zeros(N, dtype=I32, device=dev)
        self.seq_len = torch.ones(N, dtype=I32, device=dev)
        self.oshape = {'data': (N, W, eng.num_features)}
        for op in eng.ops:
            s = self.oshape[op.prev.key]
            op.alloc(self, s)
            self.oshape[op.key] = op.out_shape(s)
        keys = self.lstm_sync_keys
        if keys:
            self.lstm_arena = torch.zeros(sum(self.buf[k].numel() for k in keys), dtype=I32, device=dev)
            off = 0
            for k in keys:
                n = self.buf[k].numel()
                self.buf[k] = self.lstm_arena[off:off + n]
                off += n
        self.lstm_sync = tuple(self.buf[k] for k in keys)
        own = [k for k in self.buf if k.endswith('/w9ws')]
        if own and sum(self.buf[k].numel() for k in own) > eng.w9_defer_max_bytes and not eng.w9_flush_bytes:
            need = max(self.buf[k].numel() for k in own)
            for k in own:
                del self.buf[k]
            self.w9_hold_for.clear()
            self.buf['wgrad_ws'] = torch.empty(need, dtype=torch.uint8, device=dev)
        self.T, _, self.C = self.oshape[eng.ops[-1].key]
        self.costs = torch.zeros(N, dtype=F32, device=dev)
        _, ws_bytes, grad_shape = eng.ctc_form_of(self.C, self.T, N)
        self.ctc_grad = torch.empty(grad_shape, dtype=F32, device=dev)
        self.ctc_ws = torch.empty(ws_bytes, dtype=torch.uint8, device=dev)
        self.decoded = torch.zeros((N, self.T), dtype=I32, device=dev)
        self.decoded_len = torch.zeros(N, dtype=I32, device=dev)


class Engine(object):

    def __init__(self, net, device='cuda:0', seed=None, max_label_len=31, use_graphs=True, group=None,
                 persistent_lstm=True, fuse_conv1_pool=True, ctc_long=True, ctc_wide=True):
        from .config import cfg
        if max_label_len > self.CTC_MAX_LABEL_LEN:
            raise ValueError('max_label_len = %d: the CTC loss covers labels of at most %d characters' % (max_label_len, self.CTC_MAX_LABEL_LEN))
        if not torch.cuda.is_available():
            raise NativeError('Engine needs a ROCm GPU: the hot path has no CPU implementation')
        self.cfg = cfg
        self.net = net
        self.device = torch.device(device)
        torch.cuda.set_device(self.device)
        self.num_features = cfg.NUM_FEATURES
        self.max_label_len = max_label_len
        self.ctc_long = ctc_long
        self.ctc_wide = ctc_wide
        self.use_graphs = use_graphs
        self.persistent_lstm = persistent_lstm
        self.fuse_conv1_pool = fuse_conv1_pool
        self.fuse_bn_stats = _switch('OCR_FUSE_BN_STATS')
        self.w9_flush_bytes = int(_number('OCR_W9_FLUSH_MB', 80, float) * (1 << 20))
        self.tn_defer = _switch('OCR_TN_JOBS')
        self.tn_side = _switch('OCR_TN_SIDE', False)
        self.side_stream = torch.cuda.Stream(device=self.device) if (self.tn_side and torch.device(self.device).type == 'cuda') else None
        self.group = group
        self.world = 1
        self._check_xcd_placement()
        self.force_allreduce = bool(_env('OCR_FORCE_ALLREDUCE'))
        if group is not None or (torch.distributed.is_available() and torch.distributed.is_initialized()):
            self.world = torch.distributed.get_world_size(group)
        if _env('OCR_FAKE_WORLD'):
            self.world = _number('OCR_FAKE_WORLD', None)
            self.force_allreduce = True
        self.overlap_allreduce = _switch('OCR_OVERLAP_ALLREDUCE')
        self.dp_graph = _env('OCR_DP_GRAPH', '0') == '1'
        self.defer_w9 = _switch('OCR_W9_DEFER')
        self.w9_pair = _switch('OCR_W9_PAIR')
        self.w9_defer_max_bytes = _number('OCR_W9_DEFER_MAX_MB', self.W9_DEFER_MAX_BYTES >> 20) << 20
        self.w9_ws_pool = {}
        self.comm_stream = torch.cuda.Stream(device=self.device)
        self.dp_host_s = [0.0, 0.0, 0.0, 0.0, 0.0, 0]
        self._pack_table = None
        self._pack_table_host = None
        self._fault_hook = None
        self._watch_pending = None
        self.dropped_reports = 0
        self._lower(net)
        self._layout(net)
        self._init_params(cfg.RNG_SEED if seed is None else seed)
        self.split_op = 0
        if self.split_layer is not None:
            for i, op in enumerate(self.ops):
                if op.name == self.split_layer:
                    self.split_op = i
                    break
            for i, op in enumerate(self.ops):
                for name, owner in self._owner.items():
                    if owner == op.name:
                        assert (self.offsets[name] >= self.late_begin) == (i >= self.split_op), (op.name, name)
        self.plans = {}
        if self.dp_graph and (self.world > 1 or self.force_allreduce):
            self.dp_graph = self._check_graph_collectives()
        self.training = False
        self.train_keep_prob = 0.5
        self.scalars = torch.zeros(ops.optim_scalar_count(), dtype=torch.float64, device=self.device)
        self.opt_ready = False
        self.graph_opt = None
        self.iteration = 0
        self.refresh_weights()
        staged = getattr(net, '_staged_arrays', None)
        if staged:
            self.load_arrays(staged)

    _xcd_checked = False

    def _check_xcd_placement(self):
        if Engine._xcd_checked:
            return
        Engine._xcd_checked = True
        n = 256
        out = torch.zeros(2 * n, dtype=torch.int32, device=self.device)
        nat_call('ocr_probe_xcc', out.data_ptr(), n, 64, torch.cuda.current_stream(self.device).cuda_stream)
        xcc = out[:n].cpu().numpy()
        colocated = all(len(set(xcc[r::8].tolist())) == 1 for r in range(8))
        if not colocated:
            nat_call('ocr_set_lstm_proto', 0)

    def _layout(self, net):
        lay = FlatLayout(net.param_specs.values(), ALIGN, order=[op.name for op in self.ops])
        self._owner = lay.owner
        self.specs, self.offsets, self.n_total = lay.specs, lay.offsets, lay.n_total
        self.split_layer, self.reg_range, self.late_begin = lay.split_layer, lay.reg_range, lay.late_begin
        dev = self.device
        self.params = torch.zeros(self.n_total, dtype=F32, device=dev)
        self._grads_store = torch.zeros(self.n_total + self.GUARD_PAD, dtype=F32, device=dev)
        self.grads = self._grads_store[:self.n_total]
        self.drop_flag = self._grads_store[self.n_total:self.n_total + 1]
        self.params_bf16 = torch.zeros(self.n_total, dtype=BF16, device=dev)

    GUARD_PAD = 64

    def offset(self, name):
        return self.offsets[name]

    def _view(self, flat, name):
        s = self.specs[name]
        n = int(np.prod(s.shape))
        o = self.offsets[name]
        return flat[o:o + n].view(s.shape)

    def param(self, name):
        return self._view(self.params, name)

    def grad(self, name):
        return self._view(self.grads, name)

    def shadow(self, name):
        return self._view(self.params_bf16, name)

    def _init_params(self, seed):
        self.params.copy_(init_host_parameters(self.specs, self.offsets, self.n_total, seed))

    def load_arrays(self, arrays):
        for name, arr in arrays.items():
            t = torch.as_tensor(np.asarray(arr, np.float32))
            if tuple(t.shape) != tuple(self.specs[name].shape):
                raise ValueError('%s: shape %s does not match %s' % (name, tuple(t.shape), self.specs[name].shape))
            self.param(name).copy_(t)
        self.refresh_weights()

    def state_arrays(self):
        return {name: self.param(name).detach().cpu().numpy().copy() for name in self.specs}

    PACK_DTYPE = np.dtype([('type', '<i4'), ('R', '<i4'), ('Cc', '<i4'), ('lstm_units', '<i4'), ('ldin', '<i8'),
                           ('ldout', '<i8'), ('src', '<u8'), ('dst', '<u8'), ('n', '<i8'), ('block_start', '<i4'),
                           ('nblocks', '<i4')])

    def _build_pack_table(self):
        jobs, labels = [], []
        for op in self.ops:
            for name in op.shadow_params():
                n = int(np.prod(self.specs[name].shape))
                jobs.append(dict(type=3, src=self._view(self.params, name).reshape(-1), dst=self._view(self.params_bf16, name).reshape(-1), n=n))
                labels.append('bf16 shadow of ' + name)
        for op in self.ops:
            mine = op.pack_jobs()
            jobs.extend(mine)
            labels.extend([op.name] * len(mine))
        tab, blocks = self.pack_table(jobs)
        self.validate_pack_table(tab, blocks, labels)
        self._pack_table_host = tab
        self._pack_table = torch.from_numpy(tab.view(np.uint8).copy()).to(self.device)
        self._pack_njobs, self._pack_blocks = len(jobs), blocks

    @staticmethod
    def pack_job_blocks(j):
        t = j['type']
        if t == 0:
            return ((j['Cc'] + 63) // 64) * ((j['R'] + 63) // 64)
        if t == 1:
            return min((j['n'] + 255) // 256, 512)
        if t == 2:
            return min((j['R'] * j['Cc'] // 4 + 255) // 256, 512)
        if t == 4:
            return min((j['n'] + 255) // 256, 512)
        return min((j['n'] // 4 + 255) // 256, 2048)

    @staticmethod
    def pack_table(jobs):
        addr = lambda a: a.data_ptr() if hasattr(a, 'data_ptr') else int(a)
        tab = np.zeros(len(jobs), Engine.PACK_DTYPE)
        start = 0
        for i, j in enumerate(jobs):
            nb = Engine.pack_job_blocks(j)
            tab[i] = (j['type'], j.get('R', 0), j.get('Cc', 0), j.get('lstm_units', 0), j.get('ldin', 0), j.get('ldout', 0),
                      addr(j['src']), addr(j['dst']), j.get('n', 0), start, nb)
# ... 123 lines not shown
        d = producer.dy(sp)
        if d is None:
            return None, (lambda: None)
        owner = producer.grad_owner()
        if owner.consumers <= 1 or owner.key not in sp.dy_done:
            sp.dy_done.add(owner.key)
            return d, (lambda: None)
        tmp = self._scratch(sp, d)
        return tmp, (lambda: ops.eltwise(0, d, tmp, d))

    def grad_dst_acc(self, sp, producer, can_accumulate):
        d = producer.dy(sp)
        if d is None:
            return None, (lambda: None), False
        owner = producer.grad_owner()
        first = owner.consumers <= 1 or owner.key not in sp.dy_done
        if first or not can_accumulate:
            dst, finish = self.grad_dst(sp, producer)
            return dst, finish, False
        return d, (lambda: None), True

    def deliver(self, sp, producer, grad, mask=None):
        d = producer.dy(sp)
        if d is None:
            return
        g = grad.view(d.shape)
        if mask is None and producer.mask_in_consumer:
            mask = producer.y(sp)
        owner = producer.grad_owner()
        first = owner.consumers <= 1 or owner.key not in sp.dy_done
        sp.dy_done.add(owner.key)
        if first:
            if mask is None:
                d.copy_(g)
            else:
                ops.eltwise(2, g, mask.view(d.shape), d)
        elif mask is None:
            ops.eltwise(0, d, g, d)
        else:
            ops.eltwise(4, g, mask.view(d.shape), d)

    def plan(self, N, W):
        key = (N, W)
        if key not in self.plans:
            self.plans[key] = ShapePlan(self, N, W)
        return self.plans[key]

    def _bind(self, sp, data, seq_len, labels=None, labels_len=None):
        def as_i32(v):
            return v if torch.is_tensor(v) else torch.as_tensor(np.asarray(v, np.int32))
        sl = as_i32(seq_len)
        lab = ll = None
        if labels is not None:
            lab, ll = as_i32(labels), as_i32(labels_len)
            if lab.numel() > sp.labels.numel():
                raise ValueError('flat label vector longer than batch * max_label_len (%d)' % sp.labels.numel())
        ints = [t for t in (sl, lab, ll) if t is not None]
        if (torch.is_tensor(data) and data.is_cuda and data.dtype in (torch.uint8, F32) and data.is_contiguous()
                and data.numel() == sp.x.numel() and all(t.is_cuda and t.dtype == I32 and t.is_contiguous() for t in ints)
                and sl.numel() == sp.seq_len.numel() and (ll is None or ll.numel() == sp.labels_len.numel())):
            ops.bind_batch(data, sp.x, sl, sp.seq_len, lab, sp.labels, ll, sp.labels_len)
            return
        if torch.is_tensor(data) and data.dtype == torch.uint8:
            ops.u8_to_unit_f32(data if data.is_cuda else data.to(self.device, non_blocking=True), sp.x)
            dsts, srcs = [sp.seq_len], [sl]
        else:
            x = torch.as_tensor(np.asarray(data, np.float32)) if not torch.is_tensor(data) else data
            dsts, srcs = [sp.x, sp.seq_len], [x, sl]
        if lab is not None:
            dsts += [sp.labels[:lab.numel()], sp.labels_len]
            srcs += [lab, ll]
        for d, t in zip(dsts, srcs):
            d.copy_(t, non_blocking=True)

    def step_counter(self):
        return self.scalars[6:7]

    def _forward(self, sp, training=False):
        self.training = training
        self._zero_pending = bool(training) and self.grads.numel() % 4 == 0 and _switch('OCR_FUSE_ZERO')
        if training and not self._zero_pending:
            self.grads.zero_()
        sp.rings_ready, sp.rings_armed = set(), False
        self._ones_pending = sp.lstm_arena if (training and sp.lstm_arena is not None and _switch('OCR_FUSE_RINGFILL')) else None
        for op in self.ops:
            op.fwd(sp)
        self._ones_pending = None
        if self._zero_pending:
            self.grads.zero_()
            self._zero_pending = False

    def _loss_and_backward(self, sp, flush=True):
        sp.dy_done = set()
        sp.w9_pending = []
        sp.tn_pending = []
        sp.w9_held = None
        logits = self.ops[-1].y(sp)
        scale = ocr_dist.loss_scale(sp.N, self.world)
        path = self.ctc_form_of(sp.C, sp.T, sp.N)[0]
        if path == 'fast':
            ops.ctc_loss_train(logits, self.ops[-1].dy(sp), scale, sp.labels, sp.labels_len, sp.seq_len, self.max_label_len,
                               sp.costs, blank=0)
        elif path == 'long':
            ops.ctc_loss_long(logits, sp.labels, sp.labels_len, sp.seq_len, self.max_label_len, blank=0, want_grad=False,
                              grad_ntc_bf16=self.ops[-1].dy(sp), scale=scale, workspace=sp.ctc_ws, costs=sp.costs)
        elif path == 'wide':
            ops.ctc_loss_wide(logits, sp.labels, sp.labels_len, sp.seq_len, self.max_label_len, blank=0, want_grad=False,
                              grad_ntc_bf16=self.ops[-1].dy(sp), scale=scale, workspace=sp.ctc_ws, costs=sp.costs)
        else:
            ops.ctc_loss(logits, sp.labels, sp.labels_len, sp.seq_len, self.max_label_len, blank=0, want_grad=True,
                         workspace=sp.ctc_ws, costs=sp.costs, grads=sp.ctc_grad)
            ops.tnc_to_ntc_bf16(sp.ctc_grad, self.ops[-1].dy(sp), scale)
        for op in reversed(self.ops[self.split_op:]):
            op.bwd(sp)
        self._flush_tn(sp)
        self._join_tn(sp)
        self._release_w9(sp)
        if flush:
            self._flush_w9(sp)

    CTC_MAX_LABEL_LEN = 255

    def ctc_path_of(self, C, T):
        if ops.ctc_train_supported(C, T, self.max_label_len):
            return 'fast'
        long_covers = ops.ctc_long_supported(C, T, self.max_label_len)
        if self.ctc_long and long_covers:
            return 'long'
        if self.ctc_wide and not long_covers and ops.ctc_wide_supported(C, T, self.max_label_len):
            return 'wide'
        return 'general'

    def ctc_form_of(self, C, T, N):
        path = self.ctc_path_of(C, T)
        if path == 'wide':
            return path, ops.ctc_wide_workspace_bytes(C, self.max_label_len, T, N), (0,)
        ws_bytes = ops.ctc_workspace_bytes(self.max_label_len, T, N) if self.max_label_len <= 127 else 1
        if path == 'long':
            ws_bytes = max(ws_bytes, ops.ctc_long_workspace_bytes(C, self.max_label_len, T, N))
        return path, ws_bytes, (T, N, C)

    def ctc_path(self, N, W):
        sp = self.plan(N, W)
        return self.ctc_path_of(sp.C, sp.T)

    def _backward_early(self, sp):
        for op in reversed(self.ops[:self.split_op]):
            op.bwd(sp)
        self._flush_tn(sp)
        self._join_tn(sp)
        self._release_w9(sp)
        self._flush_w9(sp)

    def tn_push(self, sp, job, keep, fallback):
        if not self.tn_defer or not ops.gemm_tn_jobs_supported([job]):
            fallback()
            return
        sp.tn_pending.append((job, keep, fallback))
        if len(sp.tn_pending) == 2:
            self._flush_tn(sp)

    def _flush_tn(self, sp):
        pend, sp.tn_pending = sp.tn_pending, []
        if len(pend) == 2:
            if self.tn_side:
                main = torch.cuda.current_stream(self.device)
                self.side_stream.wait_stream(main)
                with torch.cuda.stream(self.side_stream):
                    ops.gemm_tn_jobs([pend[0][0], pend[1][0]])
                sp.tn_side_open = True
            else:
                ops.gemm_tn_jobs([pend[0][0], pend[1][0]])
        else:
            for _, _, fallback in pend:
                fallback()

    def _join_tn(self, sp):
        if sp.tn_side_open:
            torch.cuda.current_stream(self.device).wait_stream(self.side_stream)
            sp.tn_side_open = False

    W9_DEFER_MAX_BYTES = 192 << 20
    W9_JOB_DTYPE = np.dtype([('dw', '<u8'), ('part', '<u8'), ('dbias', '<u8'), ('cs_part', '<u8'), ('n4', '<i8'), ('slab4', '<i8'),
                             ('S', '<i4'), ('rows', '<i4'), ('Cout', '<i4'), ('block_start', '<i4')])

    def w9_append(self, sp, job, ws):
        sp.w9_pending.append(job)
        sp.w9_pending_bytes += ws.numel()
        if self.w9_flush_bytes and sp.w9_pending_bytes >= self.w9_flush_bytes:
            self._flush_w9(sp)

    def w9_hold(self, sp, key, x, dz, dw, db, ws):
        self._release_w9(sp)
        sp.w9_held = (key, x, dz, dw, db, ws)

    def _release_w9(self, sp):
        held, sp.w9_held = sp.w9_held, None
        if held is not None:
            _, x, dz, dw, db, ws = held
            job, nblk = ops.conv3x3_wgrad_deferred(x, dz, dw, db, ws)
            if job is not None:
                self.w9_append(sp, (job, nblk), ws)

    def _flush_w9(self, sp):
        self._release_w9(sp)
        pend, sp.w9_pending = sp.w9_pending, []
        sp.w9_pending_bytes = 0
        if not pend:
            return
        raw = b''.join(job for job, _ in pend)
        ent = sp.w9_tables.get(raw)
        if ent is None:
            tab = np.frombuffer(raw, dtype=self.W9_JOB_DTYPE).copy()
            assert tab.itemsize == 64 and len(tab) == len(pend)
            start = 0
            for i, (_, nblk) in enumerate(pend):
                tab['block_start'][i] = start
                start += nblk
            dev = torch.from_numpy(tab.view(np.uint8).copy()).to(self.device)
            ent = sp.w9_tables[raw] = (dev, len(pend), start)
        ops.wgrad9_reduce_jobs(*ent)

    def _capture(self, fn):
        import gc
        gc.collect()
        torch.cuda.synchronize()
        g = torch.cuda.CUDAGraph()
        was = gc.isenabled()
        gc.disable()
        try:
            with torch.cuda.graph(g, capture_error_mode='thread_local'):
                fn()
        finally:
            if was:
                gc.enable()
        return g

    def _run_split(self, sp):
        def body1():
            self._forward(sp, training=True)
            self._loss_and_backward(sp)
            self._publish_guard(sp)

        def body2():
            self._backward_early(sp)

        if not self.use_graphs:
            body1()
            return body2
        if sp.graph_fb1 is None:
            body1(); body2()
            sp.graph_fb1, sp.graph_fb2 = self._capture(body1), self._capture(body2)
        sp.graph_fb1.replay()
        return sp.graph_fb2.replay

    def _check_graph_collectives(self):
        import torch.distributed as dist
        fake = bool(_env('OCR_FAKE_WORLD'))
        if not fake:
            if not (dist.is_available() and dist.is_initialized()) or dist.get_backend(self.group) != 'nccl':
                return False
        ok = True
        try:
            t = torch.ones(256, dtype=F32, device=self.device)
            main = torch.cuda.current_stream(self.device)
            self.comm_stream.wait_stream(main)
            with torch.cuda.stream(self.comm_stream):
                ocr_dist.allreduce_sum_(t, self.group, force=self.force_allreduce)
            main.wait_stream(self.comm_stream)
            torch.cuda.synchronize()

            def body():
                cur = torch.cuda.current_stream(self.device)
                self.comm_stream.wait_stream(cur)
                with torch.cuda.stream(self.comm_stream):
                    ocr_dist.allreduce_sum_(t, self.group, force=self.force_allreduce)
                cur.wait_stream(self.comm_stream)
            g = self._capture(body)
            t.fill_(1.0)
            g.replay(); g.replay()
            torch.cuda.synchronize()
            w = float(self.world if (fake or self.world > 1) else 1)
            ok = bool(float(t[0]) == w * w and float(t[-1]) == w * w)
        except Exception as e:
            import sys
            sys.stderr.write('[engine] OCR_DP_GRAPH=1: a captured collective failed on this group (%s: %s) — three-graph schedule instead\n' % (type(e).__name__, e))
            ok = False
        if not fake and dist.get_world_size(self.group) > 1:
            v = torch.tensor([1.0 if ok else 0.0], device=self.device)
            dist.all_reduce(v, op=dist.ReduceOp.MIN, group=self.group)
            ok = bool(float(v[0]) == 1.0)
        return ok

    def _run_dp_graph(self, sp):
        if not self.opt_ready:
            self.setup_optimizer()

        def exchange(lo, hi):
            cur = torch.cuda.current_stream(self.device)
            self.comm_stream.wait_stream(cur)
            with torch.cuda.stream(self.comm_stream):
                self.allreduce_grads(lo, hi)

        def body():
            self._forward(sp, training=True)
            self._loss_and_backward(sp)
            self._publish_guard(sp)
            exchange(self.late_begin, self.n_total)
            self._backward_early(sp)
            exchange(0, self.late_begin)
            torch.cuda.current_stream(self.device).wait_stream(self.comm_stream)
            self._optim_body(None)

        if sp.graph_dp is None:
            self._guard_addrs(sp)
            self._forward(sp, training=True)
            self._loss_and_backward(sp)
            self._backward_early(sp)
            sp.graph_dp = self._capture(body)
        sp.graph_dp.replay()

    def _run_step(self, sp):
        if not self.opt_ready:
            self.setup_optimizer()

        def fb():
            self._forward(sp, training=True)
            self._loss_and_backward(sp, flush=False)
# ... 345 lines not shown
```

lstm_ctc_ocr_amd/engine_ops.py:

```python
import os

import numpy as np
import torch

from . import ops

BF16, F32, I32 = torch.bfloat16, torch.float32, torch.int32
BN_EPS = 1e-3


def _env(name, default=None):
    return os.environ.get(name, default)


def _switch(name, default=True):
    return _env(name, '1' if default else '0') != '0'


def _number(name, default, kind=int):
    return kind(_env(name, default))


def _take_ring(sp, key):
    if key not in sp.rings_ready:
# ... 275 lines not shown
        if (hasattr(self, 'wdgrad') and _switch('OCR_FUSE_UNPOOL') and isinstance(p, _PoolOp) and p.consumers == 1
                and getattr(p.prev, 'pool_after', None) is p and p.key in sp.fused_pools and p.prev.key + '/pool_codes' in sp.buf
                and ops.conv3x3_unpool_supported(s[0], s[1], s[2], self.co, self.ci, p.kw_t, p.kh_f)
                and ops.conv3x3_kernel_choice(s[0], s[1], s[2], self.co, self.ci, bias=False, relu=False) in ('conv_k3/A', 'conv_k3/D')):
            sp.unpool_pools.add(p.key)
            del sp.buf[p.key + '/dy']
        need = ops.conv3x3_wgrad_workspace_bytes(s[0], s[1], s[2], self.ci, self.co)
        have = sp.buf.get('wgrad_ws')
        if need and e.defer_w9:
            pool = e.w9_ws_pool
            have_ws = pool.get(self.key)
            if have_ws is None or have_ws.numel() < need:
                wmax = max(_number('OCR_MAX_WIDTH', 320), sp.W)
                scale = max(1, wmax // sp.W + (1 if wmax % sp.W else 0))
                big = need
                if scale > 1:
                    big = max(need, ops.conv3x3_wgrad_workspace_bytes(s[0], s[1] * scale, s[2], self.ci, self.co))
                have_ws = pool[self.key] = torch.empty(big, dtype=torch.uint8, device=dev)
            sp.buf[self.key + '/w9ws'] = have_ws[:need]
            if e.w9_pair:
                self._plan_w9_pair(sp, s)
        elif need and (have is None or have.numel() < need):
            sp.buf['wgrad_ws'] = torch.empty(need, dtype=torch.uint8, device=dev)

    def _plan_w9_pair(self, sp, s):
        e = self.eng
        i = e.ops.index(self)
        for j in range(i - 1, -1, -1):
            b = e.ops[j]
            if isinstance(b, _Conv1Op) and b.key + '/slab' in sp.buf:
                return
            if isinstance(b, _Conv3x3Op) and b.key + '/w9ws' in sp.buf:
                bs = sp.shape[b.key][0]
                if ((i >= e.split_op) == (j >= e.split_op) and b.key not in sp.w9_hold_for
                        and ops.conv3x3_wgrad_pair_supported((bs[0], bs[1], bs[2], b.ci, b.co), (s[0], s[1], s[2], self.ci, self.co))):
                    sp.w9_hold_for[self.key] = b.key
                return

    def _conv_fwd(self, sp, x, out, bias, codes):
        w, p = self.wpack.view(self.co, 3, 3, self.ci), self.pool_after
        if p is not None and p.key in sp.fused_pools:
            if codes is not None:
                ops.conv3x3_relu_pool_codes(x, w, None, p.y(sp), codes, bias, p.kw_t, p.kh_f)
            else:
                ops.conv3x3_relu_pool(x, w, out, p.y(sp), bias, p.kw_t, p.kh_f)
        elif self.bn and sp.bn_stat_rows[self.key]:
            ops.conv3x3_stats(x, w, out, sp.buf[self.key + '/bnws'], bias=bias)
        else:
            ops.conv3x3(x, w, out=out, bias=bias, relu=self.mask_in_consumer)

    def _conv_bwd(self, sp, x, dz, dw, db):
        e, o, p = self.eng, sp.shape[self.key][1], self.prev
        own_ws = sp.buf.get(self.key + '/w9ws')
        held = sp.w9_held
        if own_ws is not None and self.key in sp.w9_hold_for:
            e.w9_hold(sp, self.key, x, dz, dw, db, own_ws)
        elif own_ws is not None and held is not None and sp.w9_hold_for.get(held[0]) == self.key:
            sp.w9_held = None
            mine, theirs = ops.conv3x3_wgrad_pair_deferred((x, dz, dw, db, own_ws), held[1:])
            e.w9_append(sp, theirs, held[5])
            e.w9_append(sp, mine, own_ws)
        elif own_ws is not None:
            e._release_w9(sp)
            job, nblk = ops.conv3x3_wgrad_deferred(x, dz, dw, db, own_ws)
            if job is not None:
                e.w9_append(sp, (job, nblk), own_ws)
        else:
            ops.conv3x3_wgrad(x, dz, dw, dbias=db, workspace=sp.buf.get('wgrad_ws'))
        if p.key in sp.unpool_pools:
            pdy, finish = e.grad_dst(sp, p.prev)
            if pdy is not None:
                ops.conv3x3_dgrad_unpool(dz, self.wdgrad.view(self.ci, 3, 3, self.co), sp.buf[p.prev.key + '/pool_codes'], p.kw_t, p.kh_f,
                                         p.prev.mask_in_consumer, out=pdy)
                finish()
            return
        pdy, finish, acc = e.grad_dst_acc(sp, p, ops.conv3x3_accum_supported(o[0], o[1], o[2], self.co, self.ci))
        if pdy is not None:
            wd = self.wdgrad.view(self.ci, 3, 3, self.co)
            if sp.bn_bwd_rows.get(p.key, 0) and not acc:
                ops.conv3x3_dgrad_bnbwd(dz, wd, pdy, p.y(sp), sp.buf[p.key + '/z'], sp.buf[p.key + '/mean'], sp.buf[p.key + '/rstd'],
                                        sp.buf[p.key + '/bnws'])
            else:
                ops.conv3x3(dz, wd, out=pdy, mask=x if p.mask_in_consumer else None, accumulate=acc)
            finish()


class _Conv1x1Op(_ConvOp):
    kind = '1x1'

    def __init__(self, eng, node, prev):
        super(_Conv1x1Op, self).__init__(eng, node, prev)
        if self.ci % 8 or self.co % 8:
            raise NotImplementedError('%s: 1x1 conv needs C_in %% 8 == 0 and C_out %% 8 == 0' % self.name)
        self.wpack = torch.empty((self.co, self.ci), dtype=BF16, device=eng.device)

    def shadow_params(self):
        return [self.name + '/weights']

    def _conv_fwd(self, sp, x, out, bias, codes):
        s = sp.shape[self.key][0]
        M = s[0] * s[1] * s[2]
        ops.gemm_nt(x.view(M, self.ci), self.wpack, out=out.view(M, self.co), bias=bias, relu=self.mask_in_consumer)

    def _conv_bwd(self, sp, x, dz, dw, db):
        e, o = self.eng, sp.shape[self.key][1]
        M = o[0] * o[1] * o[2]
        pdy, finish = e.grad_dst(sp, self.prev)
        ops.gemm_tn(x.view(M, self.ci), dz.view(M, self.co), dw.view(self.ci, self.co), colsum=db)
        if pdy is not None:
            wsh = e.shadow(self.name + '/weights').view(self.ci, self.co)
            ops.gemm_nt(dz.view(M, self.co), wsh, out=pdy.view(M, self.ci),
                        mask=x.view(M, self.ci) if self.prev.mask_in_consumer else None)
            finish()


class _ConvFullOp(_ConvOp):
    kind = 'full'

    def __init__(self, eng, node, prev):
        super(_ConvFullOp, self).__init__(eng, node, prev)
        self.wpack = torch.empty((self.co, self.kh * self.kw * self.ci), dtype=BF16, device=eng.device)

    def shadow_params(self):
        return [self.name + '/weights']

    def out_shape(self, s):
        N, W, H = s[0], s[1], s[2]
        if self.kw != H:
            raise NotImplementedError('%s: VALID conv is lowered only when k_w equals the feature-axis size '
                                      '(got k_w=%d, H=%d)' % (self.name, self.kw, H))
        return (N, W - self.kh + 1, 1, self.co)

    def alloc(self, sp, s):
        super(_ConvFullOp, self).alloc(sp, s)
        N, W, H, C = s
        sp.buf[self.key + '/col'] = torch.empty((N * (W - self.kh + 1), self.kh * H * C), dtype=BF16, device=self.eng.device)
        p = self.prev
        bn = getattr(p, 'bn_fused_into', None)
        if (_switch('OCR_FUSE_COL2IM_BN', False) and isinstance(p, _PoolOp) and bn is not None and p.consumers == 1 and self.kh == 2
                and not p.mask_in_consumer and bn.key + '/pool_codes' in sp.buf and (H * C) % 8 == 0):
            sp.col_bn[bn.key] = (sp.buf[self.key + '/col'], N, W, H * C)

    def _conv_fwd(self, sp, x, out, bias, codes):
        (N, W, H, C), o = sp.shape[self.key]
        Wo = o[1]
        ops.gemm_nt(x, self.wpack, out=out.view(N * Wo, self.co), M=N * Wo, N=self.co, K=self.kh * H * C,
                    ldp=H * C, ldq=self.kh * H * C, bias=bias, relu=self.mask_in_consumer, row_group=Wo, row_skip=self.kh - 1)

    def _conv_bwd(self, sp, x, dz, dw, db):
        e, ((N, W, H, C), o) = self.eng, sp.shape[self.key]
        Wo, M, K = o[1], o[0] * o[1] * o[2], self.kh * H * C
        pdy, finish = e.grad_dst(sp, self.prev)
        dz2, dw2 = dz.view(M, self.co), dw.view(K, self.co)
        e.tn_push(sp, ops.tn_job(x, H * C, dz2, self.co, dw2, self.co, M, K, self.co, row_group=Wo, row_skip=self.kh - 1, colsum=db),
                  (x, dz2, dw2, db),
                  lambda: ops.gemm_tn(x, dz2, dw2, Mk=M, I=K, J=self.co, lda=H * C, ldb=self.co,
                                      ldo=self.co, row_group=Wo, row_skip=self.kh - 1, colsum=db))
        if pdy is not None:
            if self.prev.mask_in_consumer or self.kh != 2:
                raise NotImplementedError('%s: data gradient of a full-height VALID conv is lowered for k_h = 2 '
                                          'behind a non-ReLU producer' % self.name)
            col = sp.buf[self.key + '/col']
            wsh = e.shadow(self.name + '/weights').view(K, self.co)
            ops.gemm_nt(dz2, wsh, out=col, M=M, N=K, K=self.co)
            bn = getattr(self.prev, 'bn_fused_into', None)
            if bn is None or bn.key not in sp.col_bn:
                ops.conv5_col2im(col, pdy, N, W, H * C)
            finish()


def _conv_op(eng, node, prev):
    a = node.attrs
    if a['c_i'] == 1:
        cls = _Conv1Op
    elif (a['k_h'], a['k_w'], a['padding']) == (3, 3, 'SAME'):
        cls = _Conv3x3Op
    elif (a['k_h'], a['k_w']) == (1, 1):
        cls = _Conv1x1Op
    elif a['padding'] == 'VALID':
        cls = _ConvFullOp
    else:
        raise NotImplementedError('%s: %dx%d %s convolution is not lowered' % (node.name, a['k_h'], a['k_w'], a['padding']))
    return cls(eng, node, prev)


class _FcOp(_Conv1x1Op):

    def out_shape(self, s):
        return tuple(s[:-1]) + (self.co,)

    def alloc(self, sp, s):
        o = self.out_shape(s)
        rows = int(np.prod(s[:-1]))
        sp.shape[self.key] = ((rows, 1, 1, s[-1]), (rows, 1, 1, self.co))
        sp.buf[self.key + '/y'] = torch.empty(o, dtype=BF16, device=self.eng.device)
        sp.buf[self.key + '/dy'] = torch.empty(o, dtype=BF16, device=self.eng.device)


class _PoolOp(_Op):
    def __init__(self, eng, node, prev):
        super(_PoolOp, self).__init__(eng, node, prev)
        a = node.attrs
        self.kw_t, self.kh_f = a['k_h'], a['k_w']
        if (a['s_h'], a['s_w']) != (a['k_h'], a['k_w']) or self.kw_t not in (1, 2) or self.kh_f not in (1, 2):
            raise NotImplementedError('%s: max-pool is lowered for window == stride in {1,2}' % self.name)

    def dy_needed(self):
        return True

    def out_shape(self, s):
        N, W, H, C = s
        if W % self.kw_t or H % self.kh_f:
            raise NotImplementedError('%s: pooled axes must divide evenly (W=%d, H=%d)' % (self.name, W, H))
        return (N, W // self.kw_t, H // self.kh_f, C)

    def alloc(self, sp, s):
        o = self.out_shape(s)
        sp.shape[self.key] = (s, o)
        sp.buf[self.key + '/y'] = torch.empty(o, dtype=BF16, device=self.eng.device)
        sp.buf[self.key + '/dy'] = torch.empty(o, dtype=BF16, device=self.eng.device)

    fused_into = None
    bn_fused_into = None

    def fwd(self, sp):
        if self.bn_fused_into is not None:
            return
        if self.fused_into is None and self.key not in sp.fused_pools:
            ops.maxpool_fwd(self.prev.y(sp), self.kw_t, self.kh_f, out=self.y(sp))

    def bwd(self, sp):
        if self.fused_into is not None or self.bn_fused_into is not None or self.key in sp.unpool_pools:
            return
        pdy, finish = self.eng.grad_dst(sp, self.prev)
        if pdy is not None:
            codes = sp.buf.get(self.prev.key + '/pool_codes') if getattr(self.prev, 'pool_after', None) is self else None
            if codes is not None:
                ops.maxpool_bwd_codes(codes, self.dy(sp), self.kw_t, self.kh_f, self.prev.mask_in_consumer, out=pdy)
            else:
                ops.maxpool_bwd(self.prev.y(sp), self.dy(sp), self.kw_t, self.kh_f, self.prev.mask_in_consumer, out=pdy)
            finish()


class _ViewOp(_Op):

    def __init__(self, eng, node, prev):
        super(_ViewOp, self).__init__(eng, node, prev)
        self.mask_in_consumer = prev.mask_in_consumer

    def dy_needed(self):
        return True

    def out_shape(self, s):
        if self.node.op == 'reshape_squeeze':
            N, A, B, C = s
            return (N, A * B, C)
        return s

    def alloc(self, sp, s):
        sp.shape[self.key] = (s, self.out_shape(s))

    def y(self, sp):
        return self.prev.y(sp).view(sp.shape[self.key][1])

    def dy(self, sp):
        d = self.prev.dy(sp)
        return None if d is None else d.view(sp.shape[self.key][1])

    def grad_owner(self):
        return self.prev.grad_owner()


class _AddOp(_Op):

    def dy_needed(self):
        return True

    def out_shape(self, s):
        return s

    def alloc(self, sp, s):
        sp.shape[self.key] = (s, s)
        sp.buf[self.key + '/y'] = torch.empty(s, dtype=BF16, device=self.eng.device)
        sp.buf[self.key + '/dy'] = torch.empty(s, dtype=BF16, device=self.eng.device)

    relu = False

    fwd_by = None

    def fwd(self, sp):
        if self.fwd_by is None:
            ops.eltwise(3 if self.relu else 0, self.inputs[0].y(sp), self.inputs[1].y(sp), self.y(sp))

    def bwd(self, sp):
        for p in self.inputs:
            if getattr(p, 'mask_from', None) is self:
                continue
            self.eng.deliver(sp, p, self.dy(sp), mask=self.y(sp) if self.relu else None)


class _ReluOp(_Op):

    def dy_needed(self):
        return True

    def out_shape(self, s):
        return s

    fused_into = None

    def alloc(self, sp, s):
        sp.shape[self.key] = (s, s)
        if self.fused_into is None:
            sp.buf[self.key + '/y'] = torch.empty(s, dtype=BF16, device=self.eng.device)
            sp.buf[self.key + '/dy'] = torch.empty(s, dtype=BF16, device=self.eng.device)

    def y(self, sp):
# ... 389 lines not shown
```

lstm_ctc_ocr_amd/ops.py:

```python
import ctypes

import torch

from . import _native as nat
from ._native import EPI_ACCUM, EPI_BIAS, EPI_MASK, EPI_OUT_F32, EPI_RELU, EPI_ROWSWAP, call, ptr

BF16 = torch.bfloat16
F32 = torch.float32


def _st():
    return nat.stream()


def _dev(t):
    if not t.is_cuda:
        raise nat.NativeError("hot-path operators take device tensors only (got a CPU tensor)")
    return t


def ctc_workspace_bytes(max_label_len, max_time, minibatch):
    sz = ctypes.c_size_t(0)
    call("ocr_ctc_workspace_size", max_label_len, max_time, minibatch, ctypes.byref(sz))
    return sz.value
# ... 253 lines not shown


def gemm_nt(P, Q, out=None, *, M=None, N=None, K=None, ldp=None, ldq=None, ldo=None, bias=None, relu=False,
            out_f32=False, mask=None, accumulate=False, splits=1, row_group=0, row_skip=0, rowswap=None):
    M = P.shape[0] if M is None else M
    K = P.shape[1] if K is None else K
    N = Q.shape[0] if N is None else N
    ldp = P.stride(0) if ldp is None else ldp
    ldq = Q.stride(0) if ldq is None else ldq
    if out is None:
        out = torch.empty((M, N), dtype=F32 if out_f32 else BF16, device=P.device)
    ldo = out.stride(0) if ldo is None else ldo
    flags = 0
    if bias is not None: flags |= EPI_BIAS
    if relu: flags |= EPI_RELU
    if out.dtype == F32: flags |= EPI_OUT_F32
    if mask is not None: flags |= EPI_MASK
    if accumulate: flags |= EPI_ACCUM
    si = so = 0
    if rowswap is not None:
        flags |= EPI_ROWSWAP
        si, so = rowswap
    call("ocr_gemm_nt_bf16", ptr(_dev(P)), ldp, ptr(Q), ldq, ptr(out), ldo, M, N, K, ptr(bias), ptr(mask),
         mask.stride(0) if mask is not None else 0, flags, splits, row_group, row_skip, si, so, _st())
    return out


CONV_KERNEL_NAMES = ("gemm", "conv_halo", "conv_k2/A", "conv_k2/D", "conv_k3/A", "conv_k3/D", "conv_k3w/A", "conv_k3w/D", "conv_ws")


def conv3x3_kernel_choice(Nb, W, H, Cin, Cout, *, bias=True, relu=True, mask=False, accumulate=False, pool=(0, 0)):
    flags = (nat.EPI_BIAS if bias else 0) | (nat.EPI_RELU if relu else 0) | (nat.EPI_MASK if mask else 0) | (nat.EPI_ACCUM if accumulate else 0)
    rc = nat.lib().ocr_conv3x3_kernel_choice(int(Nb), int(W), int(H), int(Cin), int(Cout), flags, int(pool[0]), int(pool[1]))
    if rc < 0:
        raise nat.NativeError("ocr_conv3x3_kernel_choice failed: status %d (%s)" % (-rc, nat.status_string(-rc)))
    return CONV_KERNEL_NAMES[rc]


def conv3x3_accum_supported(Nb, W, H, Cin, Cout):
    return bool(nat.lib().ocr_conv3x3_accum_supported(Nb, W, H, Cin, Cout))


def conv3x3(x, wpack, out=None, *, bias=None, relu=False, mask=None, accumulate=False):
    Nb, W, H, Cin = x.shape
    Cout = wpack.shape[0]
    if out is None:
        assert not accumulate
        out = torch.empty((Nb, W, H, Cout), dtype=BF16, device=x.device)
    flags = ((EPI_BIAS if bias is not None else 0) | (EPI_RELU if relu else 0) | (EPI_MASK if mask is not None else 0) |
             (EPI_ACCUM if accumulate else 0))
    call("ocr_conv3x3_bf16", ptr(_dev(x)), ptr(wpack), ptr(out), Nb, W, H, Cin, Cout, ptr(bias), ptr(mask), flags, _st())
    return out


def conv3x3_pool_supported(Nb, W, H, Cin, Cout, kw, kh):
    return bool(nat.lib().ocr_conv3x3_pool_supported(Nb, W, H, Cin, Cout, kw, kh))


def conv3x3_relu_pool(x, wpack, out, pooled, bias, kw, kh):
    Nb, W, H, Cin = x.shape
    call("ocr_conv3x3_relu_pool_bf16", ptr(_dev(x)), ptr(wpack), ptr(out), ptr(pooled), Nb, W, H, Cin, wpack.shape[0], ptr(bias),
         kw, kh, _st())
    return out, pooled


def conv3x3_pool_codes_supported(Nb, W, H, Cin, Cout, kw, kh):
    return bool(nat.lib().ocr_conv3x3_pool_codes_supported(Nb, W, H, Cin, Cout, kw, kh))


def conv3x3_relu_pool_codes(x, wpack, out, pooled, codes, bias, kw, kh):
    Nb, W, H, Cin = x.shape
    Cout = wpack.shape[0]
    assert codes.dtype == torch.int32 and codes.numel() == Nb * (W // kw) * (H // kh) * (Cout // 8), (codes.dtype, tuple(codes.shape))
    call("ocr_conv3x3_relu_pool_codes_bf16", ptr(_dev(x)), ptr(wpack), ptr(out), ptr(pooled), ptr(codes), Nb, W, H, Cin, Cout, ptr(bias),
         kw, kh, _st())
    return out, pooled, codes


def conv3x3_unpool_supported(Nb, W, H, Cin, Cout, kw, kh):
    return bool(nat.lib().ocr_conv3x3_unpool_supported(int(Nb), int(W), int(H), int(Cin), int(Cout), int(kw), int(kh)))


def conv3x3_dgrad_unpool(dy, wdgrad, codes, kw, kh, relu_mask, out=None):
    Nb, W, H, Cin = dy.shape
    Cout = wdgrad.shape[0]
    assert codes.dtype == torch.int32 and codes.numel() == Nb * W * H * (Cout // 8), (codes.dtype, tuple(codes.shape))
    if out is None:
        out = torch.empty((Nb, W * kw, H * kh, Cout), dtype=BF16, device=dy.device)
    assert out.numel() == Nb * W * kw * H * kh * Cout
    call("ocr_conv3x3_dgrad_unpool_bf16", ptr(_dev(dy)), ptr(wdgrad), ptr(out), ptr(codes), Nb, W, H, Cin, Cout, kw, kh, int(relu_mask),
         _st())
    return out


def gemm_tn(A, B, out, *, Mk=None, I=None, J=None, lda=None, ldb=None, ldo=None, row_group=0, row_skip=0,
            a_row_off=0, scale=1.0, splits=0, colsum=None):
    Mk = B.shape[0] if Mk is None else Mk
    I = A.shape[1] if I is None else I
    J = B.shape[1] if J is None else J
    lda = A.stride(0) if lda is None else lda
    ldb = B.stride(0) if ldb is None else ldb
    ldo = out.stride(0) if ldo is None else ldo
    call("ocr_gemm_tn_bf16", ptr(_dev(A)), lda, ptr(B), ldb, ptr(out), ldo, Mk, I, J, row_group, row_skip, a_row_off,
         float(scale), splits, ptr(colsum), _st())
    return out


def gemm_tn_split_workspace(Mk, I, J):
    n = nat.lib().ocr_gemm_tn_split_workspace_floats(int(Mk), int(I), int(J))
    if n < 0:
        raise nat.NativeError("ocr_gemm_tn_split_workspace_floats: invalid shape (%d, %d, %d)" % (Mk, I, J))
    return int(n)


def gemm_tn_split(A, B, out, ws, *, colsum=None, scale=1.0):
    Mk, I, J = B.shape[0], A.shape[1], B.shape[1]
    call("ocr_gemm_tn_split_bf16", ptr(_dev(A)), A.stride(0), ptr(B), B.stride(0), ptr(out), out.stride(0), Mk, I, J, float(scale),
         ptr(colsum), ptr(ws), ws.numel(), _st())
    return out


def gemm_tn_batched(A, lda, strideA, B, ldb, strideB, out, ldo, strideOut, Mk, I, J, nbatch, colsum=None, strideColsum=0,
                    scale=1.0, splits=0):
    call("ocr_gemm_tn_batched_bf16", ptr(_dev(A)), lda, strideA, ptr(B), ldb, strideB, ptr(out), ldo, strideOut, Mk, I, J, nbatch,
         float(scale), splits, ptr(colsum), strideColsum, _st())
    return out


class TnJob(ctypes.Structure):
    _fields_ = [("A", ctypes.c_void_p), ("lda", ctypes.c_long), ("strideA", ctypes.c_long),
                ("B", ctypes.c_void_p), ("ldb", ctypes.c_long), ("strideB", ctypes.c_long),
                ("out", ctypes.c_void_p), ("ldo", ctypes.c_long), ("strideOut", ctypes.c_long),
                ("colsum", ctypes.c_void_p), ("strideColsum", ctypes.c_long),
                ("Mk", ctypes.c_int), ("I", ctypes.c_int), ("J", ctypes.c_int), ("nbatch", ctypes.c_int),
                ("row_group", ctypes.c_int), ("row_skip", ctypes.c_int), ("scale", ctypes.c_float), ("reserved", ctypes.c_int)]


def tn_job(A, lda, B, ldb, out, ldo, Mk, I, J, *, nbatch=1, strideA=0, strideB=0, strideOut=0, colsum=None, strideColsum=0, row_group=0,
           row_skip=0, scale=1.0):
    return TnJob(ptr(_dev(A)), lda, strideA, ptr(_dev(B)), ldb, strideB, ptr(out), ldo, strideOut, ptr(colsum), strideColsum,
                 Mk, I, J, nbatch, row_group, row_skip, float(scale), 0)


def gemm_tn_jobs_supported(jobs):
    arr = (TnJob * len(jobs))(*jobs)
    return bool(nat.lib().ocr_gemm_tn_jobs_supported(ctypes.cast(arr, ctypes.c_void_p), len(jobs)))


def gemm_tn_jobs(jobs):
    arr = (TnJob * len(jobs))(*jobs)
    call("ocr_gemm_tn_jobs_bf16", ctypes.cast(arr, ctypes.c_void_p), len(jobs), _st())


def lstm_xh(x2d, hout, seq_len, xh, Nb, T, D, U, ndir=2):
    call("ocr_lstm_xh", ptr(_dev(x2d)), ptr(hout), ptr(seq_len), ptr(xh), Nb, T, D, U, ndir, _st())
    return xh


def conv3x3_wgrad_workspace_bytes(Nb, W, H, Cin, Cout):
    sz = ctypes.c_size_t(0)
    call("ocr_conv3x3_wgrad_workspace_size", Nb, W, H, Cin, Cout, ctypes.byref(sz))
    return sz.value


WGRAD_KERNEL_NAMES = ("wgrad9", "wgrad9p<4>", "wgrad9p<8>", "wgrad9p<4>/zero-row", "wgrad9p<8>/zero-row", "gemm_tn2/nine-tap",
                      "gemm_tn2/paired-tap", "gemm_tn<1,4,4>", "gemm_tn<1,2,2>")


def conv3x3_wgrad_kernel_choice(Nb, W, H, Cin, Cout, *, workspace=True, splits=0):
    rc = nat.lib().ocr_conv3x3_wgrad_kernel_choice(int(Nb), int(W), int(H), int(Cin), int(Cout), int(bool(workspace)), int(splits))
    if rc < 0:
        raise nat.NativeError("ocr_conv3x3_wgrad_kernel_choice failed: status %d (%s)" % (-rc, nat.status_string(-rc)))
    return WGRAD_KERNEL_NAMES[rc & 255], rc >> 8


def conv3x3_wgrad(x, dy, dw, splits=0, dbias=None, workspace=None):
    Nb, W, H, Cin = x.shape
    Cout = dy.shape[-1]
    if workspace is not None:
        call("ocr_conv3x3_wgrad_ws_bf16", ptr(_dev(x)), ptr(dy), ptr(dw), ptr(dbias), Nb, W, H, Cin, Cout, splits,
             ptr(workspace), workspace.numel(), _st())
    else:
        call("ocr_conv3x3_wgrad_bf16", ptr(_dev(x)), ptr(dy), ptr(dw), ptr(dbias), Nb, W, H, Cin, Cout, splits, _st())
    return dw


def conv3x3_wgrad_deferred(x, dy, dw, dbias, workspace):
    Nb, W, H, Cin = x.shape
    Cout = dy.shape[-1]
    job = (ctypes.c_ubyte * 64)()
    nblk, deferred = ctypes.c_int(0), ctypes.c_int(0)
    call("ocr_conv3x3_wgrad_defer_bf16", ptr(_dev(x)), ptr(dy), ptr(dw), ptr(dbias), Nb, W, H, Cin, Cout, ptr(workspace),
         workspace.numel(), ctypes.cast(job, ctypes.c_void_p), ctypes.byref(nblk), ctypes.byref(deferred), _st())
    return (bytes(job), nblk.value) if deferred.value else (None, 0)


def conv3x3_wgrad_pair_supported(shape_first, shape_second):
    a, b = (ctypes.c_int * 5)(*[int(v) for v in shape_first]), (ctypes.c_int * 5)(*[int(v) for v in shape_second])
    rc = nat.lib().ocr_conv3x3_wgrad_pair_supported(a, b)
    if rc < 0:
        raise nat.NativeError("ocr_conv3x3_wgrad_pair_supported failed: status %d (%s)" % (-rc, nat.status_string(-rc)))
    return bool(rc)


def conv3x3_wgrad_pair_deferred(first, second):
    args, outs = [], []
    for x, dy, dw, dbias, workspace in (first, second):
        Nb, W, H, Cin = x.shape
        shape = (ctypes.c_int * 5)(Nb, W, H, Cin, dy.shape[-1])
        args += [ptr(_dev(x)), ptr(dy), ptr(dw), ptr(dbias), shape, ptr(workspace), workspace.numel()]
        outs.append(((ctypes.c_ubyte * 64)(), ctypes.c_int(0)))
    call("ocr_conv3x3_wgrad_pair_defer_bf16", *args, ctypes.cast(outs[0][0], ctypes.c_void_p), ctypes.cast(outs[1][0], ctypes.c_void_p),
         ctypes.byref(outs[0][1]), ctypes.byref(outs[1][1]), _st())
    return tuple((bytes(job), nblk.value) for job, nblk in outs)


def wgrad9_reduce_jobs(table, njobs, total_blocks):
    call("ocr_wgrad9_reduce_jobs", ptr(_dev(table)), njobs, total_blocks, _st())


def conv1_fwd(x, w, bias, relu=True, out=None):
    Nb, W, H = x.shape
    Cout = w.shape[-1]
    if out is None:
        out = torch.empty((Nb, W, H, Cout), dtype=BF16, device=x.device)
    call("ocr_conv1_fwd", ptr(_dev(x)), ptr(w), ptr(bias), ptr(out), Nb, W, H, Cout, int(relu), _st())
    return out


def conv1_wgrad(x, dz, dw, db):
    Nb, W, H = x.shape
    call("ocr_conv1_wgrad", ptr(_dev(x)), ptr(dz), ptr(dw), ptr(db), Nb, W, H, dz.shape[-1], _st())


def eltwise(op, a, b, out):
    call("ocr_eltwise_bf16", op, ptr(_dev(a)), ptr(b), ptr(out), a.numel(), _st())
    return out


def conv1_pool_fwd(x, w, bias, out=None, zero=None, codes=None, ones=None):
    Nb, W, H = x.shape
    Cout = w.shape[-1]
    if out is None:
        out = torch.empty((Nb, W // 2, H // 2, Cout), dtype=BF16, device=x.device)
    if zero is not None or codes is not None or ones is not None:
        call("ocr_conv1_pool_fwd_train", ptr(_dev(x)), ptr(w), ptr(bias), ptr(out), Nb, W, H, Cout, ptr(codes),
             ptr(_dev(zero)) if zero is not None else None, 0 if zero is None else zero.numel(),
             ptr(_dev(ones)) if ones is not None else None, 0 if ones is None else ones.numel(), _st())
    else:
        call("ocr_conv1_pool_fwd", ptr(_dev(x)), ptr(w), ptr(bias), ptr(out), Nb, W, H, Cout, _st())
    return out


def conv1_pool_bwd(x, w, bias, dp, dw, db, codes=None):
    Nb, W, H = x.shape
    if codes is not None:
        call("ocr_conv1_pool_bwd_codes", ptr(_dev(x)), ptr(w), ptr(bias), ptr(dp), ptr(dw), ptr(db), Nb, W, H, w.shape[-1], ptr(codes), _st())
    else:
        call("ocr_conv1_pool_bwd", ptr(_dev(x)), ptr(w), ptr(bias), ptr(dp), ptr(dw), ptr(db), Nb, W, H, w.shape[-1], _st())


def conv1_pool_bwd_slab_rows(Nb, W, H):
    return int(nat.lib().ocr_conv1_pool_bwd_slab_rows(int(Nb), int(W), int(H)))


def conv1_pool_bwd_slab(x, w, bias, dp, slab, codes=None):
    Nb, W, H = x.shape
    assert slab.dtype == torch.float32 and tuple(slab.shape) == (conv1_pool_bwd_slab_rows(Nb, W, H), 640)
    call("ocr_conv1_pool_bwd_slab", ptr(_dev(x)), ptr(w), ptr(bias), ptr(dp), Nb, W, H, w.shape[-1], ptr(codes), ptr(slab), _st())


def maxpool_fwd(x, kw, kh, out=None):
    Nb, W, H, C = x.shape
    if out is None:
        out = torch.empty((Nb, W // kw, H // kh, C), dtype=BF16, device=x.device)
    call("ocr_maxpool_fwd", ptr(_dev(x)), ptr(out), Nb, W, H, C, kw, kh, _st())
    return out


def maxpool_bwd(x, dy, kw, kh, relu_mask, out=None):
    Nb, W, H, C = x.shape
    if out is None:
        out = torch.empty_like(x)
    call("ocr_maxpool_bwd", ptr(_dev(x)), ptr(dy), ptr(out), Nb, W, H, C, kw, kh, int(relu_mask), _st())
    return out


def maxpool_bwd_codes(codes, dy, kw, kh, relu_mask, out=None):
    Nb, Wo, Ho, C = dy.shape
    W, H = Wo * kw, Ho * kh
    assert codes.dtype == torch.int32 and codes.numel() == Nb * Wo * Ho * (C // 8), (codes.dtype, tuple(codes.shape))
    if out is None:
        out = torch.empty((Nb, W, H, C), dtype=BF16, device=dy.device)
    call("ocr_maxpool_bwd_codes", ptr(_dev(codes)), ptr(dy), ptr(out), Nb, W, H, C, kw, kh, int(relu_mask), _st())
    return out


def bn_workspace(M, C, device):
    return torch.empty(int(nat.lib().ocr_bn_workspace_bytes(int(M), int(C))), dtype=torch.uint8, device=device)


def bn_train_fwd(x2d, gamma, beta, eps, relu, workspace, out=None, save_mean=None, save_rstd=None, residual=None, partial_rows=0,
                 pooled=None, codes=None):
    M, C = x2d.shape
    if codes is not None:
        assert pooled is not None and residual is None and out is None
# ... 274 lines not shown
```

Baseline: 59770 images/sec.

## Co-launch paired TN weight-grad jobs with NT data-grad GEMM in one kernel

Moves the igemm kernel body into a shared header so that a new combined kernel can run the two deferred TN weight-gradient jobs and the NT data-gradient GEMM of the full-height VALID conv in a single launch, split by block index. The combined path is used only when the two TN jobs together cover fewer tiles than there are CUs and leave at least a quarter of the CUs idle, so the NT blocks fill those idle CUs. This removes one kernel launch and the serialization between the under-occupied TN pair and the NT GEMM. The cost is a larger shared-LDS footprint and a register budget common to both bodies.

```diff
diff --git a/include/ocr_hip.h b/include/ocr_hip.h
--- a/include/ocr_hip.h
+++ b/include/ocr_hip.h
@@ -118,6 +118,10 @@
 } ocr_tn_job;
 int ocr_gemm_tn_jobs_supported(const ocr_tn_job* jobs, int njobs);
 int ocr_gemm_tn_jobs_bf16(const ocr_tn_job* jobs, int njobs, void* stream);
+int ocr_gemm_tn_jobs_nt_supported(const ocr_tn_job* jobs, int njobs, int M, int N, int K, int flags);
+int ocr_gemm_tn_jobs_nt_bf16(const ocr_tn_job* jobs, int njobs, const void* P, long ldp, const void* Q, long ldq, void* out, long ldo,
+                             int M, int N, int K, const float* bias, const void* mask, long ldmask, int flags, int row_group,
+                             int row_skip, int swap_inner, int swap_outer, void* stream);
 int ocr_set_wgrad_engine(int engine);
 int ocr_conv3x3_wgrad_bf16(const void* x, const void* dy, float* dw, float* dbias, int Nb, int W, int H, int Cin,
                            int Cout, int splits, void* stream);
diff --git a/lstm_ctc_ocr_amd/_native.py b/lstm_ctc_ocr_amd/_native.py
--- a/lstm_ctc_ocr_amd/_native.py
+++ b/lstm_ctc_ocr_amd/_native.py
@@ -52,6 +52,8 @@
     "ocr_gemm_tn_batched_bf16": ([_P, _L, _L, _P, _L, _L, _P, _L, _L, _I, _I, _I, _I, _F, _I, _P, _L, _P], _I),
     "ocr_gemm_tn_jobs_supported": ([_P, _I], _I),
     "ocr_gemm_tn_jobs_bf16": ([_P, _I, _P], _I),
+    "ocr_gemm_tn_jobs_nt_supported": ([_P, _I, _I, _I, _I, _I], _I),
+    "ocr_gemm_tn_jobs_nt_bf16": ([_P, _I, _P, _L, _P, _L, _P, _L, _I, _I, _I, _P, _P, _L, _I, _I, _I, _I, _I, _P], _I),
     "ocr_lstm_xh": ([_P, _P, _P, _P, _I, _I, _I, _I, _I, _P], _I),
     "ocr_set_wgrad_engine": ([_I], _I),
     "ocr_conv3x3_bf16": ([_P, _P, _P, _I, _I, _I, _I, _I, _P, _P, _I, _P], _I),
@@ -166,7 +168,7 @@
     import hashlib
     rel = [os.path.basename(f) for f in glob.glob(os.path.join(csrc, "*.hip"))]
     h = hashlib.sha256()
-    for f in sorted(rel) + ["common.h", "conv_plan.h", "ctc_common.h", "Makefile"]:
+    for f in sorted(rel) + ["common.h", "conv_plan.h", "ctc_common.h", "igemm_body.h", "Makefile"]:
         h.update(open(os.path.join(csrc, f), "rb").read())
     return h.hexdigest()[:16] + ("-exp" if experiments else "")
 
diff --git a/lstm_ctc_ocr_amd/csrc/gemm.hip b/lstm_ctc_ocr_amd/csrc/gemm.hip
--- a/lstm_ctc_ocr_amd/csrc/gemm.hip
+++ b/lstm_ctc_ocr_amd/csrc/gemm.hip
@@ -236,6 +236,7 @@
     g_use_igemm = mode != 0; g_use_halo = mode == 1; g_ig_stages = (mode == 2) ? 2 : 3;
     return OCR_OK;
 }
+bool gemm_uses_igemm() { return g_use_igemm != 0; }
 
 extern "C" int ocr_gemm_nt_bf16(const void* P, long ldp, const void* Q, long ldq, void* out, long ldo,
                                 int M, int N, int K, const float* bias, const void* mask, long ldmask,
diff --git a/lstm_ctc_ocr_amd/csrc/gemm_tn3.hip b/lstm_ctc_ocr_amd/csrc/gemm_tn3.hip
--- a/lstm_ctc_ocr_amd/csrc/gemm_tn3.hip
+++ b/lstm_ctc_ocr_amd/csrc/gemm_tn3.hip
@@ -1,4 +1,5 @@
 #include "common.h"
+#include "igemm_body.h"
 #include <stdlib.h>
 #include <type_traits>
 
@@ -232,12 +233,33 @@
     }
 }
 
+__global__ __launch_bounds__(512) __attribute__((amdgpu_waves_per_eu(2, 2))) void gemm_tn3_nt_kernel(Tn3Job j0, Tn3Job j1, IgArgs nt, int nblk0, int nblk_tn) {
+    extern __shared__ __attribute__((aligned(16))) unsigned char smem[];
+    const int bid = (int)blockIdx.x;
+    if (bid >= nblk_tn) {
+        ig_body<128, 0, 2, 8>(nt, bid - nblk_tn, smem, (const bf16_t*)tn3_zero_page);
+        return;
+    }
+    const int kh = __builtin_amdgcn_readfirstlane((int)(threadIdx.x >> 8));
+    if (bid < nblk0) {
+        if (kh == 0) tn3_body<0, 4>(j0, bid, smem); else tn3_body<1, 4>(j0, bid, smem);
+    } else {
+        if (kh == 0) tn3_body<0, 4>(j1, bid - nblk0, smem); else tn3_body<1, 4>(j1, bid - nblk0, smem);
+    }
+}
+
 static bool tn3_covers(const Tn3Job& j) {
     if (!j.A || !j.B || !j.out || j.Mk < 256 || j.I <= 0 || j.J <= 0 || (j.I & 127) || (j.J & 127) || j.nbatch < 1) return false;
     if ((j.lda & 7) || (j.ldb & 7) || (j.sA & 7) || (j.sB & 7) || ((size_t)j.A & 15) || ((size_t)j.B & 15)) return false;
     if (j.grp < 0 || j.skip < 0 || (j.grp == 0 && j.skip != 0)) return false;
     return (long)(j.I >> 7) * (j.J >> 7) * j.nbatch <= 0x7fffffL;
 }
+static int tn3_tiles(const Tn3Job& j) { return (j.I >> 7) * (j.J >> 7) * j.nbatch; }
+static int tn3_nst() {
+    static int nst = -1;
+    if (nst < 0) { const char* e = getenv("OCR_TN3_NST"); nst = (e && atoi(e) == 5) ? 5 : 4; }
+    return nst;
+}
 extern "C" int ocr_gemm_tn_jobs_supported(const void* jobs, int njobs) {
     if (!jobs || njobs < 1 || njobs > 2) return 0;
     const Tn3Job* j = (const Tn3Job*)jobs;
@@ -247,10 +269,9 @@
 extern "C" int ocr_gemm_tn_jobs_bf16(const void* jobs, int njobs, void* stream) {
     if (!ocr_gemm_tn_jobs_supported(jobs, njobs)) return OCR_ERR_INVALID;
     const Tn3Job* j = (const Tn3Job*)jobs;
-    const int t0 = (j[0].I >> 7) * (j[0].J >> 7) * j[0].nbatch;
-    const int t1 = njobs > 1 ? (j[1].I >> 7) * (j[1].J >> 7) * j[1].nbatch : 0;
-    static int nst = -1;
-    if (nst < 0) { const char* e = getenv("OCR_TN3_NST"); nst = (e && atoi(e) == 5) ? 5 : 4; }
+    const int t0 = tn3_tiles(j[0]);
+    const int t1 = njobs > 1 ? tn3_tiles(j[1]) : 0;
+    const int nst = tn3_nst();
     const int lds = nst * 2 * 64 * 256;
     if (nst == 4) {
         if (ocr_allow_lds<gemm_tn3_kernel<4>>(lds) != hipSuccess) return OCR_ERR_EXEC;
@@ -262,3 +283,37 @@
     OCR_CHECK_LAUNCH();
     return OCR_OK;
 }
+
+bool gemm_uses_igemm();
+static bool tn3_nt_pair_ok(const Tn3Job* j, int njobs, int M, int N, int K, int flags) {
+    if (!j || njobs != 2 || !tn3_covers(j[0]) || !tn3_covers(j[1]) || tn3_nst() != 4) return false;
+    if (!gemm_uses_igemm() || !ig_covers(M, N, K, flags, 0, 0) || N < 128) return false;
+    const long tiles = (long)tn3_tiles(j[0]) + tn3_tiles(j[1]);
+    const int cus = ocr_cu_count();
+    return tiles < cus && 4 * (cus - tiles) >= cus;
+}
+extern "C" int ocr_gemm_tn_jobs_nt_supported(const void* jobs, int njobs, int M, int N, int K, int flags) {
+    return tn3_nt_pair_ok((const Tn3Job*)jobs, njobs, M, N, K, flags) ? 1 : 0;
+}
+extern "C" int ocr_gemm_tn_jobs_nt_bf16(const void* jobs, int njobs, const void* P, long ldp, const void* Q, long ldq, void* out, long ldo,
+                                        int M, int N, int K, const float* bias, const void* mask, long ldmask, int flags, int row_group,
+                                        int row_skip, int swap_inner, int swap_outer, void* stream) {
+    const Tn3Job* j = (const Tn3Job*)jobs;
+    if (!P || !Q || !out || !tn3_nt_pair_ok(j, njobs, M, N, K, flags)) return OCR_ERR_INVALID;
+    if (((flags & IG_BIAS) && !bias) || ((flags & IG_MASK) && !mask)) return OCR_ERR_INVALID;
+    if ((flags & IG_ROWSWAP) && (swap_inner <= 0 || swap_outer <= 0)) return OCR_ERR_INVALID;
+    if (row_group < 0 || row_skip < 0) return OCR_ERR_INVALID;
+    IgArgs g = {};
+    g.P = (const bf16_t*)P; g.Q = (const bf16_t*)Q; g.ldp = ldp; g.ldq = ldq; g.M = M; g.N = N; g.K = K;
+    g.grp = row_group; g.skip = row_skip; g.out = out; g.ldo = ldo; g.bias = bias;
+    g.mask = (const bf16_t*)mask; g.ldmask = ldmask; g.flags = flags; g.swap_inner = swap_inner; g.swap_outer = swap_outer;
+    const int first = j[1].Mk > j[0].Mk ? 1 : 0;
+    const int t0 = tn3_tiles(j[first]), t1 = tn3_tiles(j[first ^ 1]);
+    const int nblk_nt = ((M + 255) / 256) * ((N + 127) / 128);
+    constexpr int TN_LDS = 4 * 2 * 64 * 256, NT_LDS = ig_lds_bytes<128, 2, 8>();
+    constexpr int LDS = NT_LDS > TN_LDS ? NT_LDS : TN_LDS;
+    if (ocr_allow_lds<gemm_tn3_nt_kernel>(LDS) != hipSuccess) return OCR_ERR_EXEC;
+    gemm_tn3_nt_kernel<<<t0 + t1 + nblk_nt, 512, LDS, (hipStream_t)stream>>>(j[first], j[first ^ 1], g, t0, t0 + t1);
+    OCR_CHECK_LAUNCH();
+    return OCR_OK;
+}
diff --git a/lstm_ctc_ocr_amd/csrc/igemm.hip b/lstm_ctc_ocr_amd/csrc/igemm.hip
--- a/lstm_ctc_ocr_amd/csrc/igemm.hip
+++ b/lstm_ctc_ocr_amd/csrc/igemm.hip
@@ -1,199 +1,12 @@
-#include "common.h"
+#include "igemm_body.h"
 #include <stdlib.h>
-
-enum { IG_BIAS = 1, IG_RELU = 2, IG_OUT_F32 = 4, IG_MASK = 16, IG_ROWSWAP = 32 };
-
-struct IgArgs {
-    const bf16_t* P; const bf16_t* Q;
-    long ldp, ldq;
-    int M, N, K;
-    int grp, skip;
-    int cW, cH, cC;
-    void* out; long ldo;
-    const float* bias; const bf16_t* mask; long ldmask;
-    int flags, swap_inner, swap_outer;
-};
 
 __device__ u32x4 ig_zero_page[4];
 
-typedef const __attribute__((address_space(1))) void* gptr_t;
-typedef __attribute__((address_space(3))) void* lptr_t;
-
-template <int BN, int MODE , int STAGES , int NW >
+template <int BN, int MODE, int STAGES, int NW>
 __global__ __launch_bounds__(64 * NW) __attribute__((amdgpu_waves_per_eu(2, 2))) void igemm_kernel(IgArgs g) {
-    constexpr int BM = 32 * NW, BK = 64;
-    constexpr int WAVES_N = BN / 64, WAVES_M = NW / WAVES_N;
-    constexpr int WM = BM / WAVES_M;
-    constexpr int FM = WM / 16, FN = 4;
-    constexpr int PB = BM * BK * 2, QB = BN * BK * 2, STAGE = PB + QB;
-    constexpr int QI = BN / (8 * NW);
     extern __shared__ __attribute__((aligned(16))) unsigned char smem[];
-
-    const int tid = threadIdx.x, lane = tid & 63;
-    const int wave = __builtin_amdgcn_readfirstlane(tid >> 6);
-    const int wm = wave / WAVES_N, wn = wave % WAVES_N;
-
-    const int mtiles = (g.M + BM - 1) / BM, ntiles = (g.N + BN - 1) / BN;
-    const int nblk = mtiles * ntiles;
-    int L = blockIdx.x;
-    if ((nblk & 7) == 0) L = (L & 7) * (nblk >> 3) + (L >> 3);
-    const int m0 = (L / ntiles) * BM, n0 = (L % ntiles) * BN;
-
-    const int rsub = lane >> 3;
-    const int csrc = ((lane & 7) ^ rsub) * 8;
-    const bf16_t* zero = (const bf16_t*)ig_zero_page;
-    const bf16_t* prow[4];
-    int pw[4], ph[4];
-    bool pok[4];
-#pragma unroll
-    for (int j = 0; j < 4; ++j) {
-        int m = m0 + (wave * 4 + j) * 8 + rsub;
-        pok[j] = m < g.M;
-        int mm = pok[j] ? m : 0;
-        if (MODE == 0) {
-            long phys = (long)mm + (g.grp > 0 ? (long)(mm / g.grp) * g.skip : 0);
-            prow[j] = g.P + phys * g.ldp + csrc;
-            pw[j] = ph[j] = 0;
-        } else {
-            ph[j] = mm % g.cH;
-            pw[j] = (mm / g.cH) % g.cW;
-            prow[j] = g.P + (long)mm * g.cC + csrc;
-        }
-    }
-    const bf16_t* qrow[QI];
-#pragma unroll
-    for (int j = 0; j < QI; ++j) {
-        int n = n0 + (wave * QI + j) * 8 + rsub;
-        qrow[j] = (n < g.N) ? g.Q + (long)n * g.ldq + csrc : nullptr;
-    }
-
-    auto stage_load = [&](int k0, int buf) {
-        unsigned char* sp = smem + buf * STAGE;
-        long shift = k0;
-        int dw = 0, dh = 0;
-        if (MODE == 1) {
-            int tap = k0 / g.cC;
-            dw = tap / 3 - 1; dh = tap % 3 - 1;
-            shift = ((long)dw * g.cH + dh) * g.cC + (k0 - tap * g.cC);
-        }
-#pragma unroll
-        for (int j = 0; j < 4; ++j) {
-            bool ok = pok[j];
-            if (MODE == 1) ok = ok && (unsigned)(pw[j] + dw) < (unsigned)g.cW && (unsigned)(ph[j] + dh) < (unsigned)g.cH;
-            const bf16_t* src = ok ? prow[j] + shift : zero;
-            __builtin_amdgcn_global_load_lds((gptr_t)src, (lptr_t)(sp + (wave * 4 + j) * 1024), 16, 0, 0);
-        }
-#pragma unroll
-        for (int j = 0; j < QI; ++j) {
-            const bf16_t* src = qrow[j] ? qrow[j] + k0 : zero;
-            __builtin_amdgcn_global_load_lds((gptr_t)src, (lptr_t)(sp + PB + (wave * QI + j) * 1024), 16, 0, 0);
-        }
-    };
-
-    f32x4 acc[FN][FM];
-#pragma unroll
-    for (int a = 0; a < FN; ++a)
-#pragma unroll
-        for (int b = 0; b < FM; ++b) acc[a][b] = (f32x4){0.f, 0.f, 0.f, 0.f};
-
-    const int frow = lane & 15, fq = lane >> 4, fx = lane & 7;
-    const int ntk = g.K / BK;
-    constexpr int NI = 4 + QI;
-    const unsigned lds0 = (unsigned)(size_t)(lptr_t)smem;
-    const unsigned qoff = PB + (wn * 64 + frow) * 128 + ((fq ^ fx) << 4);
-    const unsigned poff = (wm * WM + frow) * 128 + ((fq ^ fx) << 4);
-    auto compute = [&](int buf) {
-        const unsigned base = lds0 + buf * STAGE;
-        u32x4 af[2][FN], bfr[2][FM];
-#pragma unroll
-        for (int kk = 0; kk < 2; ++kk) {
-#pragma unroll
-            for (int a = 0; a < FN; ++a)
-                asm volatile("ds_read_b128 %0, %1 offset:%2" : "=v"(af[kk][a]) : "v"(base + (qoff ^ (kk * 64))), "n"(a * 2048));
-#pragma unroll
-            for (int b = 0; b < FM; ++b)
-                asm volatile("ds_read_b128 %0, %1 offset:%2" : "=v"(bfr[kk][b]) : "v"(base + (poff ^ (kk * 64))), "n"(b * 2048));
-        }
-#pragma unroll
-        for (int kk = 0; kk < 2; ++kk) {
-            if (kk == 0) asm volatile("s_waitcnt lgkmcnt(%0)" ::"n"(FN + FM) : "memory");
-            else asm volatile("s_waitcnt lgkmcnt(0)" ::: "memory");
-            __builtin_amdgcn_sched_barrier(0);
-#pragma unroll
-            for (int a = 0; a < FN; ++a)
-#pragma unroll
-                for (int b = 0; b < FM; ++b)
-                    acc[a][b] = __builtin_amdgcn_mfma_f32_16x16x32_bf16(__builtin_bit_cast(bf16x8, af[kk][a]),
-                                                                        __builtin_bit_cast(bf16x8, bfr[kk][b]), acc[a][b], 0, 0, 0);
-            __builtin_amdgcn_sched_barrier(0);
-        }
-    };
-    if (STAGES == 2) {
-        stage_load(0, 0);
-        asm volatile("s_waitcnt vmcnt(0)" ::: "memory");
-        __syncthreads();
-        for (int t = 0; t < ntk; ++t) {
-            const int cur = t & 1;
-            if (t + 1 < ntk) stage_load((t + 1) * BK, cur ^ 1);
-            compute(cur);
-            asm volatile("s_waitcnt vmcnt(0)" ::: "memory");
-            __syncthreads();
-        }
-    } else {
-        stage_load(0, 0);
-        if (ntk > 1) stage_load(BK, 1);
-        int cur = 0;
-        for (int t = 0; t < ntk; ++t) {
-            if (t + 1 < ntk) asm volatile("s_waitcnt vmcnt(%0)" ::"n"(NI) : "memory");
-            else asm volatile("s_waitcnt vmcnt(0)" ::: "memory");
-            __builtin_amdgcn_s_barrier();
-            asm volatile("" ::: "memory");
-            if (t + 2 < ntk) { int nb = cur + 2; if (nb >= 3) nb -= 3; stage_load((t + 2) * BK, nb); }
-            compute(cur);
-            asm volatile("s_waitcnt lgkmcnt(0)" ::: "memory");
-            cur = (cur == 2) ? 0 : cur + 1;
-        }
-    }
-
-    const int flags = g.flags;
-    f32x4 bv[FN];
-#pragma unroll
-    for (int a = 0; a < FN; ++a) {
-        const int n = n0 + wn * 64 + a * 16 + (lane >> 4) * 4;
-        bv[a] = (f32x4){0.f, 0.f, 0.f, 0.f};
-        if ((flags & IG_BIAS) && n < g.N) bv[a] = *(const f32x4*)(g.bias + n);
-    }
-#pragma unroll
-    for (int b = 0; b < FM; ++b) {
-        const int m = m0 + wm * WM + b * 16 + (lane & 15);
-        if (m >= g.M) continue;
-        long orow = m;
-        if (flags & IG_ROWSWAP) orow = (long)(m % g.swap_inner) * g.swap_outer + m / g.swap_inner;
-#pragma unroll
-        for (int a = 0; a < FN; ++a) {
-            const int n = n0 + wn * 64 + a * 16 + (lane >> 4) * 4;
-            if (n >= g.N) continue;
-            f32x4 v = acc[a][b] + bv[a];
-            if (flags & IG_RELU) {
-                v.x = fmaxf(v.x, 0.f); v.y = fmaxf(v.y, 0.f); v.z = fmaxf(v.z, 0.f); v.w = fmaxf(v.w, 0.f);
-            }
-            if (flags & IG_MASK) {
-                u32x2 mk = *(const u32x2*)(g.mask + (long)m * g.ldmask + n);
-                if (!(bf_lo(mk.x) > 0.f)) v.x = 0.f;
-                if (!(bf_hi(mk.x) > 0.f)) v.y = 0.f;
-                if (!(bf_lo(mk.y) > 0.f)) v.z = 0.f;
-                if (!(bf_hi(mk.y) > 0.f)) v.w = 0.f;
-            }
-            if (flags & IG_OUT_F32) {
-                *(f32x4*)((float*)g.out + orow * g.ldo + n) = v;
-            } else {
-                u32x2 pk;
-                pk.x = pack_bf2(v.x, v.y);
-                pk.y = pack_bf2(v.z, v.w);
-                *(u32x2*)((bf16_t*)g.out + orow * g.ldo + n) = pk;
-            }
-        }
-    }
+    ig_body<BN, MODE, STAGES, NW>(g, (int)blockIdx.x, smem, (const bf16_t*)ig_zero_page);
 }
 
 int g_ig_stages = 3;
@@ -201,7 +14,7 @@
 template <int BN, int MODE, int STAGES, int NW>
 static int launch_ig2(const IgArgs& g, hipStream_t stream) {
     constexpr int BM = 32 * NW;
-    constexpr int LDS = STAGES * (BM * 128 + BN * 128);
+    constexpr int LDS = ig_lds_bytes<BN, STAGES, NW>();
     if (ocr_allow_lds<igemm_kernel<BN, MODE, STAGES, NW>>(LDS) != hipSuccess) return OCR_ERR_EXEC;
     int mt = (g.M + BM - 1) / BM, nt = (g.N + BN - 1) / BN;
     igemm_kernel<BN, MODE, STAGES, NW><<<mt * nt, 64 * NW, LDS, stream>>>(g);
@@ -217,9 +30,7 @@
 int ig_try_dispatch(const void* P, long ldp, const void* Q, long ldq, void* out, long ldo, int M, int N, int K,
                     const float* bias, const void* mask, long ldmask, int flags, int mode, int grp, int skip, int cW,
                     int cH, int cC, int swap_inner, int swap_outer, hipStream_t stream) {
-    if ((K & 63) || (N & 3) || M < 1024) return -1;
-    if (mode == 1 && (cC & 63)) return -1;
-    if (flags & ~(IG_BIAS | IG_RELU | IG_OUT_F32 | IG_MASK | IG_ROWSWAP)) return -1;
+    if (!ig_covers(M, N, K, flags, mode, cC)) return -1;
     IgArgs g = {};
     g.P = (const bf16_t*)P; g.Q = (const bf16_t*)Q; g.ldp = ldp; g.ldq = ldq; g.M = M; g.N = N; g.K = K;
     g.grp = grp; g.skip = skip; g.cW = cW; g.cH = cH; g.cC = cC; g.out = out; g.ldo = ldo; g.bias = bias;
diff --git a/lstm_ctc_ocr_amd/csrc/igemm_body.h b/lstm_ctc_ocr_amd/csrc/igemm_body.h
--- /dev/null
+++ b/lstm_ctc_ocr_amd/csrc/igemm_body.h
@@ -0,0 +1,202 @@
+#pragma once
+#include "common.h"
+
+enum { IG_BIAS = 1, IG_RELU = 2, IG_OUT_F32 = 4, IG_MASK = 16, IG_ROWSWAP = 32 };
+
+struct IgArgs {
+    const bf16_t* P; const bf16_t* Q;
+    long ldp, ldq;
+    int M, N, K;
+    int grp, skip;
+    int cW, cH, cC;
+    void* out; long ldo;
+    const float* bias; const bf16_t* mask; long ldmask;
+    int flags, swap_inner, swap_outer;
+};
+
+typedef const __attribute__((address_space(1))) void* gptr_t;
+typedef __attribute__((address_space(3))) void* lptr_t;
+
+template <int BN, int STAGES, int NW>
+constexpr int ig_lds_bytes() { return STAGES * (32 * NW * 128 + BN * 128); }
+
+template <int BN, int MODE , int STAGES , int NW >
+__device__ __forceinline__ void ig_body(const IgArgs& g, const int bid, unsigned char* smem, const bf16_t* zero) {
+    constexpr int BM = 32 * NW, BK = 64;
+    constexpr int WAVES_N = BN / 64, WAVES_M = NW / WAVES_N;
+    constexpr int WM = BM / WAVES_M;
+    constexpr int FM = WM / 16, FN = 4;
+    constexpr int PB = BM * BK * 2, QB = BN * BK * 2, STAGE = PB + QB;
+    constexpr int QI = BN / (8 * NW);
+
+    const int tid = threadIdx.x, lane = tid & 63;
+    const int wave = __builtin_amdgcn_readfirstlane(tid >> 6);
+    const int wm = wave / WAVES_N, wn = wave % WAVES_N;
+
+    const int mtiles = (g.M + BM - 1) / BM, ntiles = (g.N + BN - 1) / BN;
+    const int nblk = mtiles * ntiles;
+    int L = bid;
+    if ((nblk & 7) == 0) L = (L & 7) * (nblk >> 3) + (L >> 3);
+    const int m0 = (L / ntiles) * BM, n0 = (L % ntiles) * BN;
+
+    const int rsub = lane >> 3;
+    const int csrc = ((lane & 7) ^ rsub) * 8;
+    const bf16_t* prow[4];
+    int pw[4], ph[4];
+    bool pok[4];
+#pragma unroll
+    for (int j = 0; j < 4; ++j) {
+        int m = m0 + (wave * 4 + j) * 8 + rsub;
+        pok[j] = m < g.M;
+        int mm = pok[j] ? m : 0;
+        if (MODE == 0) {
+            long phys = (long)mm + (g.grp > 0 ? (long)(mm / g.grp) * g.skip : 0);
+            prow[j] = g.P + phys * g.ldp + csrc;
+            pw[j] = ph[j] = 0;
+        } else {
+            ph[j] = mm % g.cH;
+            pw[j] = (mm / g.cH) % g.cW;
+            prow[j] = g.P + (long)mm * g.cC + csrc;
+        }
+    }
+    const bf16_t* qrow[QI];
+#pragma unroll
+    for (int j = 0; j < QI; ++j) {
+        int n = n0 + (wave * QI + j) * 8 + rsub;
+        qrow[j] = (n < g.N) ? g.Q + (long)n * g.ldq + csrc : nullptr;
+    }
+
+    auto stage_load = [&](int k0, int buf) {
+        unsigned char* sp = smem + buf * STAGE;
+        long shift = k0;
+        int dw = 0, dh = 0;
+        if (MODE == 1) {
+            int tap = k0 / g.cC;
+            dw = tap / 3 - 1; dh = tap % 3 - 1;
+            shift = ((long)dw * g.cH + dh) * g.cC + (k0 - tap * g.cC);
+        }
+#pragma unroll
+        for (int j = 0; j < 4; ++j) {
+            bool ok = pok[j];
+            if (MODE == 1) ok = ok && (unsigned)(pw[j] + dw) < (unsigned)g.cW && (unsigned)(ph[j] + dh) < (unsigned)g.cH;
+            const bf16_t* src = ok ? prow[j] + shift : zero;
+            __builtin_amdgcn_global_load_lds((gptr_t)src, (lptr_t)(sp + (wave * 4 + j) * 1024), 16, 0, 0);
+        }
+#pragma unroll
+        for (int j = 0; j < QI; ++j) {
+            const bf16_t* src = qrow[j] ? qrow[j] + k0 : zero;
+            __builtin_amdgcn_global_load_lds((gptr_t)src, (lptr_t)(sp + PB + (wave * QI + j) * 1024), 16, 0, 0);
+        }
+    };
+
+    f32x4 acc[FN][FM];
+#pragma unroll
+    for (int a = 0; a < FN; ++a)
+#pragma unroll
+        for (int b = 0; b < FM; ++b) acc[a][b] = (f32x4){0.f, 0.f, 0.f, 0.f};
+
+    const int frow = lane & 15, fq = lane >> 4, fx = lane & 7;
+    const int ntk = g.K / BK;
+    constexpr int NI = 4 + QI;
+    const unsigned lds0 = (unsigned)(size_t)(lptr_t)smem;
+    const unsigned qoff = PB + (wn * 64 + frow) * 128 + ((fq ^ fx) << 4);
+    const unsigned poff = (wm * WM + frow) * 128 + ((fq ^ fx) << 4);
+    auto compute = [&](int buf) {
+        const unsigned base = lds0 + buf * STAGE;
+        u32x4 af[2][FN], bfr[2][FM];
+#pragma unroll
+        for (int kk = 0; kk < 2; ++kk) {
+#pragma unroll
+            for (int a = 0; a < FN; ++a)
+                asm volatile("ds_read_b128 %0, %1 offset:%2" : "=v"(af[kk][a]) : "v"(base + (qoff ^ (kk * 64))), "n"(a * 2048));
+#pragma unroll
+            for (int b = 0; b < FM; ++b)
+                asm volatile("ds_read_b128 %0, %1 offset:%2" : "=v"(bfr[kk][b]) : "v"(base + (poff ^ (kk * 64))), "n"(b * 2048));
+        }
+#pragma unroll
+        for (int kk = 0; kk < 2; ++kk) {
+            if (kk == 0) asm volatile("s_waitcnt lgkmcnt(%0)" ::"n"(FN + FM) : "memory");
+            else asm volatile("s_waitcnt lgkmcnt(0)" ::: "memory");
+            __builtin_amdgcn_sched_barrier(0);
+#pragma unroll
+            for (int a = 0; a < FN; ++a)
+#pragma unroll
+                for (int b = 0; b < FM; ++b)
+                    acc[a][b] = __builtin_amdgcn_mfma_f32_16x16x32_bf16(__builtin_bit_cast(bf16x8, af[kk][a]),
+                                                                        __builtin_bit_cast(bf16x8, bfr[kk][b]), acc[a][b], 0, 0, 0);
+            __builtin_amdgcn_sched_barrier(0);
+        }
+    };
+    if (STAGES == 2) {
+        stage_load(0, 0);
+        asm volatile("s_waitcnt vmcnt(0)" ::: "memory");
+        __syncthreads();
+        for (int t = 0; t < ntk; ++t) {
+            const int cur = t & 1;
+            if (t + 1 < ntk) stage_load((t + 1) * BK, cur ^ 1);
+            compute(cur);
+            asm volatile("s_waitcnt vmcnt(0)" ::: "memory");
+            __syncthreads();
+        }
+    } else {
+        stage_load(0, 0);
+        if (ntk > 1) stage_load(BK, 1);
+        int cur = 0;
+        for (int t = 0; t < ntk; ++t) {
+            if (t + 1 < ntk) asm volatile("s_waitcnt vmcnt(%0)" ::"n"(NI) : "memory");
+            else asm volatile("s_waitcnt vmcnt(0)" ::: "memory");
+            __builtin_amdgcn_s_barrier();
+            asm volatile("" ::: "memory");
+            if (t + 2 < ntk) { int nb = cur + 2; if (nb >= 3) nb -= 3; stage_load((t + 2) * BK, nb); }
+            compute(cur);
+            asm volatile("s_waitcnt lgkmcnt(0)" ::: "memory");
+            cur = (cur == 2) ? 0 : cur + 1;
+        }
+    }
+
+    const int flags = g.flags;
+    f32x4 bv[FN];
+#pragma unroll
+    for (int a = 0; a < FN; ++a) {
+        const int n = n0 + wn * 64 + a * 16 + (lane >> 4) * 4;
+        bv[a] = (f32x4){0.f, 0.f, 0.f, 0.f};
+        if ((flags & IG_BIAS) && n < g.N) bv[a] = *(const f32x4*)(g.bias + n);
+    }
+#pragma unroll
+    for (int b = 0; b < FM; ++b) {
+        const int m = m0 + wm * WM + b * 16 + (lane & 15);
+        if (m >= g.M) continue;
+        long orow = m;
+        if (flags & IG_ROWSWAP) orow = (long)(m % g.swap_inner) * g.swap_outer + m / g.swap_inner;
+#pragma unroll
+        for (int a = 0; a < FN; ++a) {
+            const int n = n0 + wn * 64 + a * 16 + (lane >> 4) * 4;
+            if (n >= g.N) continue;
+            f32x4 v = acc[a][b] + bv[a];
+            if (flags & IG_RELU) {
+                v.x = fmaxf(v.x, 0.f); v.y = fmaxf(v.y, 0.f); v.z = fmaxf(v.z, 0.f); v.w = fmaxf(v.w, 0.f);
+            }
+            if (flags & IG_MASK) {
+                u32x2 mk = *(const u32x2*)(g.mask + (long)m * g.ldmask + n);
+                if (!(bf_lo(mk.x) > 0.f)) v.x = 0.f;
+                if (!(bf_hi(mk.x) > 0.f)) v.y = 0.f;
+                if (!(bf_lo(mk.y) > 0.f)) v.z = 0.f;
+                if (!(bf_hi(mk.y) > 0.f)) v.w = 0.f;
+            }
+            if (flags & IG_OUT_F32) {
+                *(f32x4*)((float*)g.out + orow * g.ldo + n) = v;
+            } else {
+                u32x2 pk;
+                pk.x = pack_bf2(v.x, v.y);
+                pk.y = pack_bf2(v.z, v.w);
+                *(u32x2*)((bf16_t*)g.out + orow * g.ldo + n) = pk;
+            }
+        }
+    }
+}
+
+static inline bool ig_covers(int M, int N, int K, int flags, int mode, int cC) {
+    if ((K & 63) || (N & 3) || M < 1024) return false;
+    if (mode == 1 && (cC & 63)) return false;
+    return !(flags & ~(IG_BIAS | IG_RELU | IG_OUT_F32 | IG_MASK | IG_ROWSWAP));
+}
diff --git a/lstm_ctc_ocr_amd/engine.py b/lstm_ctc_ocr_amd/engine.py
--- a/lstm_ctc_ocr_amd/engine.py
+++ b/lstm_ctc_ocr_amd/engine.py
@@ -103,6 +103,7 @@
         self.w9_flush_bytes = int(_number('OCR_W9_FLUSH_MB', 80, float) * (1 << 20))
         self.tn_defer = _switch('OCR_TN_JOBS')
         self.tn_side = _switch('OCR_TN_SIDE', False)
+        self.tn_nt_pair = _switch('OCR_TN_NT_PAIR')
         self.side_stream = torch.cuda.Stream(device=self.device) if (self.tn_side and torch.device(self.device).type == 'cuda') else None
         self.group = group
         self.world = 1
@@ -532,17 +533,22 @@
         self._release_w9(sp)
         self._flush_w9(sp)
 
-    def tn_push(self, sp, job, keep, fallback):
+    def tn_push(self, sp, job, keep, fallback, nt=None):
         if not self.tn_defer or not ops.gemm_tn_jobs_supported([job]):
             fallback()
-            return
+            return False
         sp.tn_pending.append((job, keep, fallback))
         if len(sp.tn_pending) == 2:
-            self._flush_tn(sp)
-
-    def _flush_tn(self, sp):
+            return self._flush_tn(sp, nt)
+        return False
+
+    def _flush_tn(self, sp, nt=None):
         pend, sp.tn_pending = sp.tn_pending, []
         if len(pend) == 2:
+            jobs = [pend[0][0], pend[1][0]]
+            if nt is not None and self.tn_nt_pair and not self.tn_side and ops.gemm_tn_jobs_nt_supported(jobs, nt[3], nt[4], nt[5]):
+                ops.gemm_tn_jobs_nt(jobs, nt[0], nt[1], nt[2], M=nt[3], N=nt[4], K=nt[5])
+                return True
             if self.tn_side:
                 main = torch.cuda.current_stream(self.device)
                 self.side_stream.wait_stream(main)
@@ -554,6 +560,7 @@
         else:
             for _, _, fallback in pend:
                 fallback()
+        return False
 
     def _join_tn(self, sp):
         if sp.tn_side_open:
diff --git a/lstm_ctc_ocr_amd/engine_ops.py b/lstm_ctc_ocr_amd/engine_ops.py
--- a/lstm_ctc_ocr_amd/engine_ops.py
+++ b/lstm_ctc_ocr_amd/engine_ops.py
@@ -451,17 +451,21 @@
         Wo, M, K = o[1], o[0] * o[1] * o[2], self.kh * H * C
         pdy, finish = e.grad_dst(sp, self.prev)
         dz2, dw2 = dz.view(M, self.co), dw.view(K, self.co)
-        e.tn_push(sp, ops.tn_job(x, H * C, dz2, self.co, dw2, self.co, M, K, self.co, row_group=Wo, row_skip=self.kh - 1, colsum=db),
-                  (x, dz2, dw2, db),
-                  lambda: ops.gemm_tn(x, dz2, dw2, Mk=M, I=K, J=self.co, lda=H * C, ldb=self.co,
-                                      ldo=self.co, row_group=Wo, row_skip=self.kh - 1, colsum=db))
+        nt = None
+        if pdy is not None and not self.prev.mask_in_consumer and self.kh == 2:
+            col = sp.buf[self.key + '/col']
+            wsh = e.shadow(self.name + '/weights').view(K, self.co)
+            nt = (dz2, wsh, col, M, K, self.co)
+        paired = e.tn_push(sp, ops.tn_job(x, H * C, dz2, self.co, dw2, self.co, M, K, self.co, row_group=Wo, row_skip=self.kh - 1, colsum=db),
+                           (x, dz2, dw2, db),
+                           lambda: ops.gemm_tn(x, dz2, dw2, Mk=M, I=K, J=self.co, lda=H * C, ldb=self.co,
+                                               ldo=self.co, row_group=Wo, row_skip=self.kh - 1, colsum=db), nt=nt)
         if pdy is not None:
-            if self.prev.mask_in_consumer or self.kh != 2:
+            if nt is None:
                 raise NotImplementedError('%s: data gradient of a full-height VALID conv is lowered for k_h = 2 '
                                           'behind a non-ReLU producer' % self.name)
-            col = sp.buf[self.key + '/col']
-            wsh = e.shadow(self.name + '/weights').view(K, self.co)
-            ops.gemm_nt(dz2, wsh, out=col, M=M, N=K, K=self.co)
+            if not paired:
+                ops.gemm_nt(dz2, wsh, out=col, M=M, N=K, K=self.co)
             bn = getattr(self.prev, 'bn_fused_into', None)
             if bn is None or bn.key not in sp.col_bn:
                 ops.conv5_col2im(col, pdy, N, W, H * C)
diff --git a/lstm_ctc_ocr_amd/ops.py b/lstm_ctc_ocr_amd/ops.py
--- a/lstm_ctc_ocr_amd/ops.py
+++ b/lstm_ctc_ocr_amd/ops.py
@@ -429,6 +429,24 @@
     call("ocr_gemm_tn_jobs_bf16", ctypes.cast(arr, ctypes.c_void_p), len(jobs), _st())
 
 
+def gemm_tn_jobs_nt_supported(jobs, M, N, K, flags=0):
+    arr = (TnJob * len(jobs))(*jobs)
+    return bool(nat.lib().ocr_gemm_tn_jobs_nt_supported(ctypes.cast(arr, ctypes.c_void_p), len(jobs), int(M), int(N), int(K), int(flags)))
+
+
+def gemm_tn_jobs_nt(jobs, P, Q, out, *, M=None, N=None, K=None, ldp=None, ldq=None, ldo=None, row_group=0, row_skip=0):
+    M = P.shape[0] if M is None else M
+    K = P.shape[1] if K is None else K
+    N = Q.shape[0] if N is None else N
+    ldp = P.stride(0) if ldp is None else ldp
+    ldq = Q.stride(0) if ldq is None else ldq
+    ldo = out.stride(0) if ldo is None else ldo
+    arr = (TnJob * len(jobs))(*jobs)
+    call("ocr_gemm_tn_jobs_nt_bf16", ctypes.cast(arr, ctypes.c_void_p), len(jobs), ptr(_dev(P)), ldp, ptr(Q), ldq, ptr(out), ldo, M, N, K,
+         None, None, 0, EPI_OUT_F32 if out.dtype == F32 else 0, row_group, row_skip, 0, 0, _st())
+    return out
+
+
 def lstm_xh(x2d, hout, seq_len, xh, Nb, T, D, U, ndir=2):
     call("ocr_lstm_xh", ptr(_dev(x2d)), ptr(hout), ptr(seq_len), ptr(xh), Nb, T, D, U, ndir, _st())
     return xh
```

Result: faster. 60770 images/sec, median of 6 (+1.7%).
